# oksuman/sorting-fhe

Hardware: AMD Instinct MI355X
Metric: encrypted rank-sort homomorphic comparisons/s (N^2 per DirectSort<N>::sort) (higher is better)
Workload: dtype u64 (RNS residues, 40/60-bit primes); 1 GPU; directsort_n256_2e16; N=256, ring_dim=65536, mult_depth=34, scale_bits=40, parallelism=replicas x1

## Files before the change

include/sfhe.h:

```cpp
#ifndef SFHE_H
#define SFHE_H

#include <stddef.h>
#include <stdint.h>

#ifdef __cplusplus
extern "C" {
#endif

#define SFHE_ABI_VERSION 3

#define SFHE_OK 0
#define SFHE_EINVAL (-1)
#define SFHE_ESCHEME (-2)
#define SFHE_EDEVICE (-3)
#define SFHE_ENOTIMPL (-4)

typedef struct sfhe_ctx sfhe_ctx;
typedef struct sfhe_ct sfhe_ct;
typedef struct sfhe_sorter sfhe_sorter;

#define SFHE_FLEXIBLEAUTO 2
#define SFHE_FLEXIBLEAUTOEXT 3

// ... 4 lines not shown
    uint32_t mult_depth;
    uint32_t scaling_mod_size;
    uint32_t first_mod_size;
    uint32_t batch_size;
    uint32_t ring_dim;
    int32_t security_level;
    uint32_t num_large_digits;
    int32_t device;
    uint64_t seed;
    int32_t scaling_technique;
} sfhe_params;

int sfhe_abi_version(void);
const char* sfhe_last_error(void);
const char* sfhe_backend(void);
void sfhe_params_default(sfhe_params* p);

int sfhe_context_create(const sfhe_params* p, sfhe_ctx** out);
void sfhe_context_destroy(sfhe_ctx* c);
int sfhe_keygen(sfhe_ctx* c);
int sfhe_rotate_keygen(sfhe_ctx* c, const int32_t* idx, size_t count);
int sfhe_context_info(sfhe_ctx* c, uint32_t* ring_dim, uint32_t* mult_depth, uint32_t* num_q,
                      uint32_t* num_p, uint32_t* dnum);
int sfhe_context_primes(sfhe_ctx* c, uint64_t* out, size_t cap, size_t* count);
int sfhe_set_plaintext_cache(sfhe_ctx* c, int on);
int sfhe_set_quiet(sfhe_ctx* c, int quiet);
int sfhe_sync(sfhe_ctx* c);
int sfhe_op_stats(sfhe_ctx* c, uint64_t* counts, double* bytes, int reset);
int sfhe_bootstrap_graphs(sfhe_ctx* c, uint64_t* count);
int sfhe_encode_counts(sfhe_ctx* c, uint64_t* device, uint64_t* host);
int sfhe_decode_counts(sfhe_ctx* c, uint64_t* device, uint64_t* host);
int sfhe_tie_counts(sfhe_ctx* c, uint64_t* fused, uint64_t* composed);
int sfhe_const_term_counts(sfhe_ctx* c, uint64_t* merged, uint64_t* single, uint64_t* composed);
int sfhe_sample_counts(sfhe_ctx* c, uint64_t* device, uint64_t* host);
int sfhe_pool_bytes(sfhe_ctx* c, uint64_t* bytes);
int sfhe_live_contexts(void);
#define SFHE_KFAM_NTT 0
#define SFHE_KFAM_CONV 1
#define SFHE_KFAM_KSINNER 2
#define SFHE_KFAM_NTTKS 3
#define SFHE_KFAM_OTHER 4
#define SFHE_KFAM_ALL 5
int sfhe_kernel_timing(sfhe_ctx* c, uint32_t family, uint32_t period);
int sfhe_kernel_timing_read(sfhe_ctx* c, uint32_t family, uint64_t* launches, uint64_t* timed,
                            double* ms, double* bytes);
int sfhe_serialize_lanes(sfhe_ctx* c, int on);
int sfhe_stack_stats(sfhe_ctx* c, uint64_t* merged, uint64_t* single);
int sfhe_comm_stats_reset(sfhe_ctx* c, int timed);
int sfhe_comm_stats(sfhe_ctx* c, uint64_t* calls, double* bytes, double* ms);

int sfhe_encrypt(sfhe_ctx* c, const double* values, size_t len, uint32_t slots, uint32_t level,
                 sfhe_ct** out);
int sfhe_encrypt_batch(sfhe_ctx* c, const double* values, size_t stride, const size_t* lens, size_t count,
                       uint32_t slots, const uint32_t* levels, sfhe_ct** outs);
int sfhe_decrypt(sfhe_ctx* c, const sfhe_ct* ct, double* out, size_t cap, size_t* len);
int sfhe_decrypt_batch(sfhe_ctx* c, const sfhe_ct* const* cts, size_t count, double* out, size_t stride,
                       size_t* lens);
void sfhe_ct_free(sfhe_ct* ct);
int sfhe_ct_clone(const sfhe_ct* ct, sfhe_ct** out);
int sfhe_ct_info(const sfhe_ct* ct, uint32_t* level, uint32_t* slots, uint32_t* limbs);
int sfhe_ct_set_slots(sfhe_ct* ct, uint32_t slots);
int sfhe_ct_download(sfhe_ctx* c, const sfhe_ct* ct, uint64_t* out, size_t cap_words);

int sfhe_eval_add(sfhe_ctx* c, const sfhe_ct* a, const sfhe_ct* b, sfhe_ct** out);
int sfhe_eval_sub(sfhe_ctx* c, const sfhe_ct* a, const sfhe_ct* b, sfhe_ct** out);
int sfhe_eval_add_const(sfhe_ctx* c, const sfhe_ct* a, double k, sfhe_ct** out);
int sfhe_eval_mult_const(sfhe_ctx* c, const sfhe_ct* a, double k, sfhe_ct** out);
int sfhe_eval_mult_plain(sfhe_ctx* c, const sfhe_ct* a, const double* values, size_t len,
                         uint32_t slots, sfhe_ct** out);
int sfhe_eval_mult(sfhe_ctx* c, const sfhe_ct* a, const sfhe_ct* b, sfhe_ct** out);
int sfhe_eval_rotate(sfhe_ctx* c, const sfhe_ct* a, int32_t r, sfhe_ct** out);
int sfhe_eval_rotate_sum(sfhe_ctx* c, const sfhe_ct* const* a, const int32_t* r, size_t count, sfhe_ct** out);
int sfhe_bootstrap_setup(sfhe_ctx* c, uint32_t budget_c2s, uint32_t budget_s2c, uint32_t slots);
int sfhe_bootstrap_depth(sfhe_ctx* c, uint32_t budget_c2s, uint32_t budget_s2c, uint32_t slots, uint32_t* depth);
int sfhe_bootstrap(sfhe_ctx* c, const sfhe_ct* a, uint32_t iterations, uint32_t precision, sfhe_ct** out);
int sfhe_eval_chebyshev(sfhe_ctx* c, const sfhe_ct* x, const double* coeffs, size_t count,
                        double a, double b, sfhe_ct** out);

int sfhe_sign(sfhe_ctx* c, const sfhe_ct* x, int n, int dg, int df, sfhe_ct** out);
int sfhe_compare(sfhe_ctx* c, const sfhe_ct* a, const sfhe_ct* b, int n, int dg, int df,
                 sfhe_ct** out);
int sfhe_direct_sort_params(uint32_t N, uint32_t* mult_depth, int32_t* rotations, size_t cap,
                            size_t* count);
int sfhe_doubled_sinc_coeffs(uint32_t N, double* out, size_t cap, size_t* count);
int sfhe_sorter_create(sfhe_ctx* c, uint32_t N, int debug, sfhe_sorter** out);
int sfhe_sorter_create_rot(sfhe_ctx* c, uint32_t N, int debug, const int32_t* rotations, size_t nrot,
                           sfhe_sorter** out);
void sfhe_sorter_destroy(sfhe_sorter* s);
int sfhe_sorter_sort(sfhe_sorter* s, sfhe_ct* in, int n, int dg, int df, sfhe_ct** out);
int sfhe_sorter_rank(sfhe_sorter* s, const sfhe_ct* in, int n, int dg, int df, sfhe_ct** out);
int sfhe_sorter_place(sfhe_sorter* s, const sfhe_ct* rank, sfhe_ct* in, sfhe_ct** out);
int sfhe_sorter_sort_stable(sfhe_sorter* s, sfhe_ct* in, int n, int dg, int df, sfhe_ct** out);
int sfhe_sorter_rank_stable(sfhe_sorter* s, const sfhe_ct* in, int n, int dg, int df, sfhe_ct** out);
int sfhe_sorter_graph_nodes(const sfhe_sorter* s, uint64_t* nodes);
int sfhe_sorter_graph_ntt_time(sfhe_sorter* s, int reps, double* ms, uint64_t* launches, double* bytes);
int sfhe_sorter_graph_family_time(sfhe_sorter* s, uint32_t family, int reps, double* ms, uint64_t* launches,
                                  double* bytes);
int sfhe_sorter_sort_hybrid1(sfhe_sorter* s, sfhe_ct* in, int n, int dg, int df, sfhe_ct** out);
int sfhe_hybrid1_params(uint32_t N, uint32_t* mult_depth, int32_t* rotations, size_t cap, size_t* count);

int sfhe_sorter_sort_hybrid(sfhe_sorter* s, sfhe_ct* in, int variant, int n, int dg, int df, sfhe_ct** out);
int sfhe_hybrid_params(uint32_t N, int variant, uint32_t* mult_depth, int32_t* rotations, size_t cap,
                       size_t* count);
int sfhe_sorter_place_2n(sfhe_sorter* s, const sfhe_ct* rank, sfhe_ct* in, sfhe_ct** out);
int sfhe_sorter_sort_bitonic(sfhe_sorter* s, sfhe_ct* in, int n, int dg, int df, sfhe_ct** out);
// ... 39 lines not shown
```

sorting-fhe_amd/csrc/algo/sign.cpp:

```cpp
#include "sign.h"

#include <algorithm>
#include <cmath>
#include <cstdlib>
#include <map>
#include <vector>

using namespace lbcrypto;

namespace {

using Ct = Ciphertext<DCRTPoly>;

Ct constTermAt(const CryptoContext<DCRTPoly>& cc, const Ct& x, double c, uint32_t at) {
    const uint64_t *r0, *r1;
    std::vector<DeviceBufferPtr> keep;
    cc->RowsAt(x, at - 1, &r0, &r1, keep);
    const std::vector<const uint64_t*> i0{r0}, i1{r1};
    const std::vector<double> w{c}, sc{x->scale};
    return cc->LinearWSumRescale(i0, i1, w, at - 1, x->GetSlots(), &sc);
}

struct OddPoly {
    const CryptoContext<DCRTPoly>& cc;
// ... 18 lines not shown
        if (cnt == 1) return x->GetLevel() + 1;
        const size_t half = cnt / 2;
        return std::max(natural(half), pw[powIndex(half)]->GetLevel()) + 1;
    }
    Ct eval(const double* c, size_t cnt, uint32_t want) {
        if (cnt == 1) return constAt(c[0], std::max(x->GetLevel() + 1, want));
        const size_t half = cnt / 2, j = powIndex(half);
        const uint32_t Lp = std::max(std::max(natural(half), pw[j]->GetLevel()) + 1, want);
        Ct hi = eval(c + half, half, Lp - 1);
        Ct prod = cc->EvalMult(hi, power(j, Lp - 1));
        Ct lo = eval(c, half, Lp);
        return cc->EvalAdd(lo, prod);
    }
};

bool signBatch() {
    static const bool on = [] {
        const char* v = std::getenv("SFHE_SIGN_BATCH");
        return !v || *v != '0';
    }();
    return on;
}

struct OddPolyWaves {
    const CryptoContext<DCRTPoly>& cc;
    const Ct& x;
    const uint32_t L;
    struct Node {
        const double* c;
        size_t cnt, j;
        uint32_t Lp;
        int hi, lo;
        Ct prod, out;
    };
    std::vector<Node> nodes;
    std::vector<Ct> pw;
    std::map<std::pair<size_t, uint32_t>, Ct> aligned;

    uint32_t pwLevel(size_t j) const { return L + 1 + (uint32_t)j; }
    uint32_t natural(size_t cnt) const {
        if (cnt == 1) return L + 1;
        const size_t half = cnt / 2;
        return std::max(natural(half), pwLevel(OddPoly::powIndex(half))) + 1;
    }
    int build(const double* c, size_t cnt, uint32_t want) {
        Node nd{c, cnt, 0, 0, -1, -1, nullptr, nullptr};
        if (cnt == 1) {
            nd.Lp = std::max(L + 1, want);
        } else {
            const size_t half = cnt / 2;
            nd.j = OddPoly::powIndex(half);
            nd.Lp = std::max(std::max(natural(half), pwLevel(nd.j)) + 1, want);
            nd.hi = build(c + half, half, nd.Lp - 1);
            nd.lo = build(c, half, nd.Lp);
        }
        nodes.push_back(nd);
        return (int)nodes.size() - 1;
    }
    Ct run(const std::vector<double>& c) {
        const int root = build(c.data(), c.size(), 0);
        size_t npw = 1;
        for (size_t p = 4; p < 2 * c.size(); p *= 2) ++npw;
        cc->Settle(x);
        while (!nodes[root].out) {
            std::vector<Ct> prods;
            const size_t ready = pw.size();
            if (pw.size() < npw) {
                pw.push_back(cc->EvalSquare(pw.empty() ? x : pw.back()));
                prods.push_back(pw.back());
            }
            std::vector<std::pair<size_t, uint32_t>> align;
            for (Node& nd : nodes) {
                if (nd.cnt == 1 || nd.prod || nd.j >= ready) continue;
                const Ct* power = &pw[nd.j];
                if (pwLevel(nd.j) < nd.Lp - 1) {
                    const auto key = std::make_pair(nd.j, nd.Lp - 1);
                    auto it = aligned.find(key);
                    if (it == aligned.end()) {
                        if (std::find(align.begin(), align.end(), key) == align.end()) align.push_back(key);
                        continue;
                    }
                    power = &it->second;
                }
                if (!nodes[nd.hi].out) continue;
                nd.prod = cc->EvalMult(nodes[nd.hi].out, *power);
                prods.push_back(nd.prod);
            }
            const bool first = ready == 0;
            if (prods.empty() && align.empty() && !first)
                throw OpenFHEException("internal: odd-polynomial wave evaluation stalled");
            cc->MaterializeMany(prods, std::vector<char>(prods.size(), 0));
            if (first) {
                std::vector<std::pair<double, uint32_t>> terms;
                for (const Node& nd : nodes)
                    if (nd.cnt == 1) terms.emplace_back(nd.c[0], nd.Lp);
                const auto cts = cc->ConstTermsRescale(x, terms);
                size_t t = 0;
                for (Node& nd : nodes)
                    if (nd.cnt == 1) nd.out = cts[t++];
            }
            for (const auto& key : align) aligned[key] = cc->AdjustLevel(pw[key.first], key.second);
            for (Node& nd : nodes)
                if (nd.cnt > 1 && !nd.out && nd.prod && nodes[nd.lo].out) nd.out = cc->EvalAdd(nodes[nd.lo].out, nd.prod);
        }
        return nodes[root].out;
    }
};

Ct oddPolyFull(const CryptoContext<DCRTPoly>& cc, const Ct& x, const std::vector<double>& c) {
    if (signBatch() && c.size() > 1) {
        OddPolyWaves w{cc, x, x->GetLevel(), {}, {}, {}};
        return w.run(c);
    }
    std::vector<Ct> pw;
    pw.push_back(cc->EvalSquare(x));
    for (size_t p = 4; p < 2 * c.size(); p *= 2) pw.push_back(cc->EvalSquare(pw.back()));
    OddPoly op{cc, x, pw, {}};
    return op.eval(c.data(), c.size(), 0);
}

template <int n>
struct CompositePolys;

template <>
struct CompositePolys<3> {
    static constexpr int g_depth = 3, f_depth = 3;
    static Ct g(const Ct& x, const CryptoContext<DCRTPoly>& cc) {
        static const std::vector<double> c = {4589.0 / 1024, -16577.0 / 1024, 25614.0 / 1024,
                                              -12860.0 / 1024};
        return oddPolyFull(cc, x, c);
    }
    static Ct f(const Ct& x, const CryptoContext<DCRTPoly>& cc) {
        static const std::vector<double> c = {35.0 / 16, -35.0 / 16, 21.0 / 16, -5.0 / 16};
        return oddPolyFull(cc, x, c);
    }
};
// ... 58 lines not shown
```

sorting-fhe_amd/csrc/capi.cpp:

```cpp
#include <cstring>
#include <fstream>
#include <iostream>
#include <memory>
#include <mutex>
#include <sstream>
#include <streambuf>
#include <string>

#include "../../include/sfhe.h"
#include "algo/coefficients.h"
#include "algo/comparison.h"
#include "algo/encryption.h"
#include "algo/rotation.h"
#include "algo/sign.h"
#include "algo/sort_algo.h"
#include "algo/kway_adapter.h"
#include "core/openfhe.h"
#include "core/state.h"

using namespace lbcrypto;
using Ct = Ciphertext<DCRTPoly>;

struct sfhe_ctx {
    CryptoContext<DCRTPoly> cc;
// ... 322 lines not shown
        for (size_t k = 0; k < count; ++k) {
            const auto& v = pts[k]->GetRealPackedValue();
            if (lens) lens[k] = v.size();
            for (size_t i = 0; i < v.size() && i < stride; ++i) out[k * stride + i] = v[i];
        }
    });
}

int sfhe_decode_counts(sfhe_ctx* c, uint64_t* device, uint64_t* host) {
    REQUIRE(c && device && host, "null argument");
    auto s = c->cc->GetOpStats();
    *device = s.dev_decodes;
    *host = s.host_decodes;
    return SFHE_OK;
}

int sfhe_tie_counts(sfhe_ctx* c, uint64_t* fused, uint64_t* composed) {
    REQUIRE(c && fused && composed, "null argument");
    auto s = c->cc->GetOpStats();
    *fused = s.tie_fused;
    *composed = s.tie_composed;
    return SFHE_OK;
}

int sfhe_const_term_counts(sfhe_ctx* c, uint64_t* merged, uint64_t* single, uint64_t* composed) {
    REQUIRE(c && merged && single && composed, "null argument");
    auto s = c->cc->GetOpStats();
    *merged = s.const_merged;
    *single = s.const_single;
    *composed = s.const_composed;
    return SFHE_OK;
}

void sfhe_ct_free(sfhe_ct* ct) { delete ct; }

int sfhe_ct_clone(const sfhe_ct* ct, sfhe_ct** out) {
    REQUIRE(ct && out, "null argument");
    return guard([&] { *out = wrap(ct->ct->Clone()); });
}

int sfhe_ct_info(const sfhe_ct* ct, uint32_t* level, uint32_t* slots, uint32_t* limbs) {
    REQUIRE(ct, "null ciphertext");
    if (level) *level = ct->ct->GetLevel();
    if (slots) *slots = ct->ct->GetSlots();
    if (limbs) *limbs = ct->ct->GetNumLimbs();
    return SFHE_OK;
}

int sfhe_ct_set_slots(sfhe_ct* ct, uint32_t slots) {
    REQUIRE(ct && slots && !(slots & (slots - 1)), "slots must be a power of two");
    ct->ct->SetSlots(slots);
    return SFHE_OK;
}

int sfhe_ct_download(sfhe_ctx* c, const sfhe_ct* ct, uint64_t* out, size_t cap) {
    REQUIRE(c && ct && out, "null argument");
    const size_t n = c->cc->GetRingDimension();
    const size_t L = ct->ct->GetNumLimbs();
    REQUIRE(cap >= 2 * L * n, "output buffer too small");
    return guard([&] { c->cc->DownloadRows(ct->ct, out); });
}

#define BINOP(name, expr)                                                           \
    int name(sfhe_ctx* c, const sfhe_ct* a, const sfhe_ct* b, sfhe_ct** out) {       \
        REQUIRE(c && a && b && out, "null argument");                               \
        return guard([&] { *out = wrap(expr); });                                   \
    }
BINOP(sfhe_eval_add, c->cc->EvalAdd(a->ct, b->ct))
BINOP(sfhe_eval_sub, c->cc->EvalSub(a->ct, b->ct))
BINOP(sfhe_eval_mult, c->cc->EvalMult(a->ct, b->ct))

int sfhe_eval_add_const(sfhe_ctx* c, const sfhe_ct* a, double k, sfhe_ct** out) {
    REQUIRE(c && a && out, "null argument");
    return guard([&] { *out = wrap(c->cc->EvalAdd(a->ct, k)); });
}
int sfhe_eval_mult_const(sfhe_ctx* c, const sfhe_ct* a, double k, sfhe_ct** out) {
    REQUIRE(c && a && out, "null argument");
    return guard([&] { *out = wrap(c->cc->EvalMult(a->ct, k)); });
}
int sfhe_eval_mult_plain(sfhe_ctx* c, const sfhe_ct* a, const double* v, size_t len,
                         uint32_t slots, sfhe_ct** out) {
    REQUIRE(c && a && out && (v || !len), "null argument");
    return guard([&] {
        auto pt = c->cc->MakeCKKSPackedPlaintext(std::vector<double>(v, v + len), 1,
                                                 a->ct->GetLevel(), nullptr, slots);
        *out = wrap(c->cc->EvalMult(a->ct, pt));
    });
}
int sfhe_eval_rotate(sfhe_ctx* c, const sfhe_ct* a, int32_t r, sfhe_ct** out) {
    REQUIRE(c && a && out, "null argument");
    return guard([&] { *out = wrap(c->cc->EvalRotate(a->ct, r)); });
}
int sfhe_eval_rotate_sum(sfhe_ctx* c, const sfhe_ct* const* a, const int32_t* r, size_t count, sfhe_ct** out) {
    REQUIRE(c && a && r && out && count, "null argument");
    for (size_t k = 0; k < count; ++k) REQUIRE(a[k], "null argument");
    return guard([&] {
        std::vector<Ciphertext<DCRTPoly>> v;
        for (size_t k = 0; k < count; ++k) v.push_back(a[k]->ct);
        *out = wrap(c->cc->EvalRotateSum(v, std::vector<int32_t>(r, r + count)));
    });
}
int sfhe_bootstrap_setup(sfhe_ctx* c, uint32_t budget_c2s, uint32_t budget_s2c, uint32_t slots) {
    REQUIRE(c, "null argument");
    REQUIRE(c->keys.secretKey, "sfhe_keygen must be called first");
    return guard([&] {
        c->cc->EvalBootstrapSetup({budget_c2s, budget_s2c}, {0, 0}, slots);
        c->cc->EvalBootstrapKeyGen(c->keys.secretKey, slots);
    });
}
int sfhe_bootstrap_depth(sfhe_ctx* c, uint32_t budget_c2s, uint32_t budget_s2c, uint32_t slots, uint32_t* depth) {
    REQUIRE(c && depth, "null argument");
    return guard([&] { *depth = c->cc->GetBootstrapDepth({budget_c2s, budget_s2c}, slots); });
}
int sfhe_bootstrap(sfhe_ctx* c, const sfhe_ct* a, uint32_t iterations, uint32_t precision, sfhe_ct** out) {
    REQUIRE(c && a && out, "null argument");
    return guard([&] { *out = wrap(c->cc->EvalBootstrap(a->ct, iterations, precision)); });
}
int sfhe_eval_chebyshev(sfhe_ctx* c, const sfhe_ct* x, const double* coeffs, size_t count,
                        double a, double b, sfhe_ct** out) {
    REQUIRE(c && x && coeffs && count && out, "null argument");
    return guard([&] {
        *out = wrap(c->cc->EvalChebyshevSeriesPS(x->ct, std::vector<double>(coeffs, coeffs + count), a, b));
    });
}

int sfhe_sign(sfhe_ctx* c, const sfhe_ct* x, int n, int dg, int df, sfhe_ct** out) {
    REQUIRE(c && x && out, "null argument");
    REQUIRE(n == 3 || n == 4, "composite sign degree n must be 3 or 4");
    return guard([&] { *out = wrap(sign(x->ct, c->cc, SignFunc::CompositeSign, cfgOf(n, dg, df))); });
}

int sfhe_compare(sfhe_ctx* c, const sfhe_ct* a, const sfhe_ct* b, int n, int dg, int df,
// ... 546 lines not shown
```

sorting-fhe_amd/csrc/core/chebyshev.cpp:

```cpp
#include <algorithm>
#include <cmath>
#include <cstdio>
#include <cstdlib>
#include <map>

#include "state.h"

namespace lbcrypto {

uint32_t ChebyshevPSDepth(uint32_t d) {
    if (d <= 1) return 1;
    if (d == 2) return 2;
    static const uint32_t ub[] = {5, 13, 27, 59, 119, 247, 495, 1007, 2031, 4031, 8127, 16255, 32511, 65023};
    for (uint32_t i = 0; i < sizeof(ub) / sizeof(ub[0]); ++i)
        if (d <= ub[i]) return 3 + i;
    SFHE_THROW("Chebyshev degree too large");
}

std::vector<double> EvalChebyshevCoefficients(std::function<double(double)> func, double a,
                                              double b, uint32_t degree) {
    if (!degree) SFHE_THROW("degree must be positive");
    const double bMinusA = 0.5 * (b - a), bPlusA = 0.5 * (b + a);
    const double piByDeg = M_PI / (double)degree;
    std::vector<double> fx(degree);
// ... 15 lines not shown
    });
    return c;
}

namespace {

using Ct = Ciphertext<DCRTPoly>;
using Addend = CryptoContextImpl<DCRTPoly>::MultAddend;

struct Val {
    bool isConst = true;
    double c = 0.0;
    Ct ct;
    int node = -1;
};

bool psWaves() {
    static const bool on = [] {
        const char* v = std::getenv("SFHE_PS_WAVES");
        return !v || *v != '0';
    }();
    return on;
}

class PSEvaluator {
  public:
    PSEvaluator(CryptoContextImpl<DCRTPoly>* cc, const Ct& y, uint32_t l, uint32_t D)
        : cc(cc), l(l), k(1u << l), D(D) {
        T.resize(k + 1);
        T[1] = y;
        for (uint32_t half = 1; half < k; half *= 2) {
            const uint32_t lo = half + 1, hi = std::min(k, 2 * half);
            std::vector<Ct> as, bs;
            for (uint32_t j = lo; j <= hi; ++j) {
                as.push_back(doubled(j / 2));
                bs.push_back(j % 2 == 0 ? T[j / 2] : T[j / 2 + 1]);
            }
            uint32_t top = 0;
            for (size_t i = 0; i < as.size(); ++i) top = std::max(top, std::max(as[i]->GetLevel(), bs[i]->GetLevel()) + 1);
            if (psFma() && top <= cc->GetMultiplicativeDepth()) {
                std::vector<Addend> adds;
                for (uint32_t j = lo; j <= hi; ++j) {
                    const uint32_t lv = std::max(as[j - lo]->GetLevel(), bs[j - lo]->GetLevel()) + 1;
                    adds.push_back(j % 2 == 0 ? Addend{nullptr, 1, -1.0} : Addend{atLevel(1, lv), -1, 0.0});
                }
                if (psWaves()) {
                    auto ts = cc->EvalMultManyAdd(as, bs, adds);
                    for (uint32_t j = lo; j <= hi; ++j) T[j] = ts[j - lo];
                } else {
                    for (uint32_t j = lo; j <= hi; ++j) T[j] = cc->EvalMultAdd(as[j - lo], bs[j - lo], adds[j - lo]);
                }
                continue;
            }
            std::vector<Ct> prods;
            if (psWaves()) {
                prods = cc->EvalMultMany(as, bs);
            } else {
                for (size_t i = 0; i < as.size(); ++i) prods.push_back(cc->EvalMult(as[i], bs[i]));
            }
            for (uint32_t j = lo; j <= hi; ++j) {
                const Ct& prod = prods[j - lo];
                T[j] = (j % 2 == 0) ? cc->EvalAdd(prod, -1.0) : cc->EvalSub(prod, atLevel(1, prod->GetLevel()));
            }
        }
        giant[l] = T[k];
    }

    void precomputeLeaves(const std::vector<double>& p, uint32_t depth) {
        std::vector<std::pair<std::vector<double>, uint32_t>> leaves;
        plan(p, depth, 0, leaves);
        std::map<uint32_t, std::vector<size_t>> byLevel;
        for (size_t i = 0; i < leaves.size(); ++i) byLevel[leaves[i].second].push_back(i);
        pre.assign(leaves.size(), nullptr);
        preConst.assign(leaves.size(), 0);
        for (auto& kv : byLevel) {
            const uint32_t L = kv.first;
            std::vector<uint32_t> js;
            for (uint32_t j = 1; j <= k; ++j)
                for (size_t i : kv.second)
                    if (j < leaves[i].first.size() && leaves[i].first[j] != 0.0) {
                        js.push_back(j);
                        break;
                    }
            std::vector<const uint64_t*> ins0, ins1;
            std::vector<double> sc;
            std::vector<DeviceBufferPtr> keep;
            for (uint32_t j : js) {
                const Ct& t = T[j];
                const uint64_t *r0, *r1;
                cc->RowsAt(t, L, &r0, &r1, keep);
                ins0.push_back(r0);
// ... 224 lines not shown

    int leafSumLevel(const std::vector<double>& p, uint32_t want) const {
        if (naturalOnly()) want = 0;
        int lev = -1;
        for (uint32_t j = 1; j < p.size(); ++j)
            if (p[j] != 0.0) lev = std::max(lev, (int)T[j]->GetLevel());
        if (lev < 0) return -1;
        return std::max(lev, (int)want - 1);
    }

    static bool naturalOnly() {
        static const bool on = [] {
            const char* v = std::getenv("SFHE_PS_NATURAL");
            return v && *v == '1';
        }();
        return on;
    }

    static void trim(std::vector<double>& p) {
        while (!p.empty() && p.back() == 0.0) p.pop_back();
    }

    uint32_t powerLevel(uint32_t M) const {
        if (M <= k) return T[M]->GetLevel();
        return powerLevel(M / 2) + 1;
    }

    const Ct& power(uint32_t M) {
        if (M <= k) return T[M];
        uint32_t i = (uint32_t)__builtin_ctz(M);
        auto it = giant.find(i);
        if (it != giant.end()) return it->second;
        const Ct& half = power(M / 2);
        const Ct twice = cc->EvalAdd(half, half);
        return giant[i] = cc->EvalMultAdd(twice, half, Addend{nullptr, 1, -1.0});
    }

    const Ct& doubled(uint32_t j) {
        auto it = twice.find(j);
        if (it != twice.end()) return it->second;
        return twice[j] = cc->EvalAdd(T[j], T[j]);
    }

    const Ct& alignedPower(uint32_t M, uint32_t level) {
        const Ct& t = power(M);
        if (t->GetLevel() >= level) return t;
        auto key = std::make_pair(M, level);
        auto it = alignedPow.find(key);
        if (it != alignedPow.end()) return it->second;
        return alignedPow[key] = cc->AdjustLevel(t, level);
    }

    const Ct& atLevel(uint32_t j, uint32_t level) {
        auto key = std::make_pair(j, level);
        auto it = aligned.find(key);
        if (it != aligned.end()) return it->second;
        return aligned[key] = (T[j]->GetLevel() == level ? T[j] : cc->AdjustLevel(T[j], level));
    }

    Val leaf(const std::vector<double>& p, uint32_t want) {
        if (!pre.empty()) {
            bool any = false;
            for (uint32_t j = 1; j < p.size(); ++j) any = any || p[j] != 0.0;
            if (!any) return Val{true, p[0], nullptr};
            if (nextLeaf >= pre.size()) SFHE_THROW("internal: Chebyshev leaf plan mismatch");
            Val out;
            out.isConst = false;
            out.ct = pre[nextLeaf];
            const bool constIn = preConst[nextLeaf];
            pre[nextLeaf++] = nullptr;
            if (p[0] != 0.0 && !constIn) out.ct = cc->EvalAdd(out.ct, p[0]);
            return out;
        }
        const int lv = leafSumLevel(p, want);
// ... 2 lines not shown
        std::vector<double> w, sc;
        std::vector<DeviceBufferPtr> keep;
        for (uint32_t j = 1; j < p.size(); ++j) {
            if (p[j] == 0.0) continue;
            const Ct& t = T[j];
            const uint64_t *r0, *r1;
            cc->RowsAt(t, (uint32_t)lv, &r0, &r1, keep);
            ins0.push_back(r0);
            ins1.push_back(r1);
            w.push_back(p[j]);
            sc.push_back(t->scale);
        }
        Val out;
        out.isConst = false;
        out.ct = cc->LinearWSumRescale(ins0, ins1, w, (uint32_t)lv, T[1]->GetSlots(), &sc, p[0]);
        return out;
    }

    CryptoContextImpl<DCRTPoly>* cc;
    uint32_t l, k, D;
    std::vector<Ct> pre;
    std::vector<char> preConst;
    size_t nextLeaf = 0;
    std::vector<Ct> T;
    std::map<uint32_t, Ct> giant;
    std::map<std::pair<uint32_t, uint32_t>, Ct> aligned, alignedPow;
    std::map<uint32_t, Ct> twice;
};

void psDebugCounts(const CryptoContextImpl<DCRTPoly>* cc, const char* where) {
    if (!std::getenv("SFHE_PS_DEBUG")) return;
    uint64_t sums = 0, consts = 0, pairs = 0;
    cc->FusedSumCounts(&sums, &consts, &pairs);
    std::fprintf(stderr, "PSFMA %s | fused sums %llu | fused constants %llu | paired weighted sums %llu\n", where,
                 (unsigned long long)sums, (unsigned long long)consts, (unsigned long long)pairs);
}

}

Ciphertext<DCRTPoly> CryptoContextImpl<DCRTPoly>::EvalChebyshevSeriesPS(
    const Ciphertext<DCRTPoly>& x, const std::vector<double>& coeffs, double a, double b) {
    OpLock g(st.get());
    static const bool lazyPs = [] {
        const char* v = std::getenv("SFHE_LAZY_PS");
        return v && *v == '1';
    }();
    struct Hold {
        SfheContextState* s;
        bool on;
        ~Hold() {
            if (on) --s->lazyHold;
        }
    } hold{st.get(), !lazyPs};
    if (hold.on) ++st->lazyHold;
    std::vector<double> p(coeffs);
    while (!p.empty() && p.back() == 0.0) p.pop_back();
    if (p.empty()) SFHE_THROW("empty Chebyshev series");
    p[0] *= 0.5;
    Ciphertext<DCRTPoly> y = x;
    if (a != -1.0 || b != 1.0) {
        y = EvalMult(x, 2.0 / (b - a));
        y = EvalAdd(y, -(a + b) / (b - a));
    }
    const uint32_t d = (uint32_t)p.size() - 1;
    if (d == 0) return EvalAdd(EvalMult(y, 0.0), p[0]);
    const uint32_t D = ChebyshevPSDepth(d);
    uint32_t bestL = 1;
    double bestCost = 1e300;
// ... 112 lines not shown
```

sorting-fhe_amd/csrc/core/context.cpp:

```cpp
#include <typeindex>
#include <tuple>
#include <algorithm>
#include <atomic>
#include <cmath>
#include <cstdio>
#include <cstdlib>
#include <cstring>
#include <random>

#include "state.h"

namespace lbcrypto {

namespace {

u64 mulmod(u64 a, u64 b, u64 m) { return (u64)((u128)a * b % m); }
u64 powmod(u64 a, u64 e, u64 m) {
    u64 r = 1 % m;
    a %= m;
    while (e) {
        if (e & 1) r = mulmod(r, a, m);
        a = mulmod(a, a, m);
        e >>= 1;
    }
// ... 851 lines not shown
        const uint32_t ell = s->ellOf(level);
        if (ell < 2) SFHE_THROW("no levels left to rescale (multiplicative depth exhausted)");
        if (s->shardAt(ell)) {
            keySwitchShard(cc, d2, ell, s->relinKey, d0, d1, 1, 1);
            return rescale(cc, d0, d1, level, slots);
        }
        const DeviceBufferPtr& key = s->relinFor(ell);
        const int tier = key->ksTier;
        const uint32_t n = s->n, K = s->Kof(tier);
        const uint32_t beta = (ell + s->alpha - 1) / s->alpha;
        const size_t stride = (size_t)(ell + K) * n;
        auto acc = s->alloc(2 * stride);
        const int rowDone = modupInner(cc, acc->ptr, d2, ell, key, d0, d1, s->pModQof(tier)[ell - 1], 0, ell - 1);
        Ct out = newCt(cc, level + 1, slots);
        auto scratch = s->alloc((size_t)2 * (ell - 1) * n);
        if (f && *f && sfp_moddown_rescale_add &&
            sfp_moddown_rescale_add(s->dev, out->c0, out->c1, d0, d1, acc->ptr, stride, ell, K, s->Lq,
                                    s->moddownConvOf(tier), s->pInvModQof(tier), s->pModQof(tier),
                                    s->qInvTable[ell].data(), scratch->ptr, rowDone, f->r0, f->r1, f->sign,
                                    f->cst) == 0)
            f->done = true;
        else
            sfp_moddown_rescale(s->dev, out->c0, out->c1, d0, d1, acc->ptr, stride, ell, K, s->Lq,
                                s->moddownConvOf(tier), s->pInvModQof(tier), s->pModQof(tier),
                                s->qInvTable[ell].data(), scratch->ptr, rowDone);
        s->stats.keyswitch++;
        s->stats.rescale++;
        s->countBytes((3.0 * ell + 2.0 * beta * (ell + K)) * n * 8);
        s->countBytes(4.0 * ell * n * 8);
        return out;
    }

    static Ct multRelinRescale(CC* cc, const uint64_t* a0, const uint64_t* a1, const uint64_t* b0,
                               const uint64_t* b1, uint32_t level, uint32_t slots, Fma* f = nullptr) {
        SfheContextState* s = cc->st.get();
        const uint32_t ell = s->ellOf(level);
        if (ell < 2) SFHE_THROW("no levels left to rescale (multiplicative depth exhausted)");
        const size_t pw = s->polyWords(level);
        if (!s->shardAt(ell)) {
            const DeviceBufferPtr& key = s->relinFor(ell);
            const int tier = key->ksTier;
            const uint32_t n = s->n, K = s->Kof(tier), beta = (ell + s->alpha - 1) / s->alpha;
            const size_t stride = (size_t)(ell + K) * n;
            Ct out = newCt(cc, level + 1, slots);
            auto acc = s->alloc(2 * stride);
            auto ext = s->alloc(stride * beta);
            auto scratch = s->alloc((size_t)2 * ell * n);
            auto& convs = modupConv(cc, ell, tier);
            int rc = -1;
            if (f && *f && sfp_mult_relin_rescale_add) {
                rc = sfp_mult_relin_rescale_add(s->dev, out->c0, out->c1, a0, a1, b0, b1, ell, K, s->Lq, s->alpha,
                                                convs.data(), key->ptr, s->moddownConvOf(tier),
                                                s->pInvModQof(tier), s->pModQof(tier), s->qInvTable[ell].data(),
                                                acc->ptr, ext->ptr, scratch->ptr, f->r0, f->r1, f->sign, f->cst);
                if (rc == 0) f->done = true;
            }
            if (rc != 0)
                rc = sfp_mult_relin_rescale(s->dev, out->c0, out->c1, a0, a1, b0, b1, ell, K, s->Lq, s->alpha,
                                            convs.data(), key->ptr, s->moddownConvOf(tier), s->pInvModQof(tier),
                                            s->pModQof(tier), s->qInvTable[ell].data(), acc->ptr, ext->ptr,
                                            scratch->ptr);
            if (rc == 0) {
                s->stats.keyswitch++;
                s->stats.rescale++;
                s->countBytes((3.0 * ell + 2.0 * beta * (ell + K)) * n * 8);
                s->countBytes(4.0 * ell * n * 8);
                return out;
            }
        }
        auto t = s->alloc(3 * pw);
        uint64_t* d0 = t->ptr;
        uint64_t* d1 = d0 + pw;
        uint64_t* d2 = d1 + pw;
        sfp_tensor(s->dev, d0, d1, d2, a0, a1, b0, b1, s->qmap(ell));
        return relinRescale(cc, d0, d1, d2, level, slots, f);
    }

    static std::vector<Ct> multRelinRescaleMany(CC* cc, const std::vector<const CiphertextImpl<DCRTPoly>*>& a,
                                                const std::vector<const CiphertextImpl<DCRTPoly>*>& b, uint32_t level,
                                                const std::vector<uint32_t>& slots, std::vector<Fma>* fs = nullptr) {
        SfheContextState* s = cc->st.get();
        const size_t cnt = a.size();
        const uint32_t ell = s->ellOf(level);
        std::vector<Ct> out(cnt);
        if (ell < 2) SFHE_THROW("no levels left to rescale (multiplicative depth exhausted)");
        const DeviceBufferPtr& key = s->relinFor(ell);
        const int tier = key->ksTier;
        const uint32_t n = s->n, K = s->Kof(tier), beta = (ell + s->alpha - 1) / s->alpha;
        const size_t stride = (size_t)(ell + K) * n;
        auto& convs = modupConv(cc, ell, tier);
        size_t done = 0;
        {
        BatchScope bs(cc, s->shardAt(ell) ? 0 : (uint32_t)cnt);
        if (bs) {
            for (; done < cnt; ++done) {
                out[done] = newCt(cc, level + 1, slots[done]);
                auto acc = s->alloc(2 * stride);
                auto ext = s->alloc(stride * beta);
                auto scratch = s->alloc((size_t)2 * ell * n);
                bs.lane((uint32_t)done);
                Fma* f = fs && (*fs)[done] ? &(*fs)[done] : nullptr;
                int rc = -1;
                if (f && sfp_mult_relin_rescale_add) {
                    rc = sfp_mult_relin_rescale_add(s->dev, out[done]->c0, out[done]->c1, a[done]->c0, a[done]->c1,
                                                    b[done]->c0, b[done]->c1, ell, K, s->Lq, s->alpha, convs.data(),
                                                    key->ptr, s->moddownConvOf(tier), s->pInvModQof(tier),
                                                    s->pModQof(tier), s->qInvTable[ell].data(), acc->ptr, ext->ptr,
                                                    scratch->ptr, f->r0, f->r1, f->sign, f->cst);
                    if (rc == 0) f->done = true;
                }
                if (rc != 0)
                    rc = sfp_mult_relin_rescale(s->dev, out[done]->c0, out[done]->c1, a[done]->c0, a[done]->c1,
                                                b[done]->c0, b[done]->c1, ell, K, s->Lq, s->alpha, convs.data(),
                                                key->ptr, s->moddownConvOf(tier), s->pInvModQof(tier),
                                                s->pModQof(tier), s->qInvTable[ell].data(), acc->ptr, ext->ptr,
                                                scratch->ptr);
                if (rc != 0) break;
                s->stats.keyswitch++;
                s->stats.rescale++;
                s->countBytes((3.0 * ell + 2.0 * beta * (ell + K)) * n * 8);
                s->countBytes(4.0 * ell * n * 8);
            }
        }
        }
        for (size_t i = done; i < cnt; ++i)
            out[i] = multRelinRescale(cc, a[i]->c0, a[i]->c1, b[i]->c0, b[i]->c1, level, slots[i],
                                      fs ? &(*fs)[i] : nullptr);
        return out;
    }

    static void innerAndModDown(CC* cc, const uint64_t* ext, size_t stride, uint32_t beta,
                                uint32_t ell, const DeviceBufferPtr& key, uint64_t* out0,
                                uint64_t* out1, int add0, int add1, uint32_t gal = 0) {
        SfheContextState* s = cc->st.get();
        if (s->shardAt(ell)) {
            if (gal) SFHE_THROW("internal: a permuted inner product at a sharded level");
            return innerModDownShard(s, ext, stride, beta, ell, key, out0, out1, add0, add1);
        }
        const int tier = key->ksTier;
        const uint32_t n = s->n, K = s->Kof(tier);
        const size_t accStride = (size_t)(ell + K) * n;
        if (stride != accStride) SFHE_THROW("internal: extended digits of another special-prime tier");
        auto acc = s->alloc(2 * accStride);
        if (gal)
            sfp_ks_inner_aut(s->dev, acc->ptr, acc->ptr + accStride, ext, stride, key->ptr, beta, ell, K, s->Lq, gal);
        else
            sfp_ks_inner(s->dev, acc->ptr, acc->ptr + accStride, ext, stride, key->ptr, beta, ell, K, s->Lq);
        auto scratch = s->alloc((size_t)2 * ell * n);
        sfp_moddown2(s->dev, out0, out1, acc->ptr, accStride, ell, K, s->Lq, s->moddownConvOf(tier),
                     s->pInvModQof(tier), add0, add1, scratch->ptr, 0);
    }

    static std::vector<sfp_conv*>& modupConv(CC* cc, uint32_t ell, int tier = -1) {
        SfheContextState* s = cc->st.get();
        auto& cache = tier < 0 ? s->modupConv : s->tiers[(size_t)tier].modupConv;
        auto it = cache.find(ell);
        if (it != cache.end()) return it->second;
        std::vector<sfp_conv*> v;
        const uint32_t K = s->Kof(tier);
        uint32_t beta = (ell + s->alpha - 1) / s->alpha;
// ... 643 lines not shown
        for (size_t g : grp) {
            used[g] = true;
            defs.push_back(SfheInternal::takeDeferred(*a[idx[g]], true));
            auto* m = static_cast<DeferredMacPlain*>(defs.back().get());
            for (auto& b : m->pins) s->dep(b.get());
            pts.insert(pts.end(), m->pts.begin(), m->pts.end());
        }
        SfheInternal::encodeBatch(cc, pts, level);
        std::vector<const uint64_t*> mm;
        for (auto& p : pts) mm.push_back(SfheInternal::encoded(cc, p, level));
        const uint32_t ell = s->ellOf(level);
        const size_t pw = s->polyWords(level);
        std::vector<DeviceBufferPtr> bufs;
        std::vector<uint64_t*> o0, o1;
        for (uint32_t g = 0; g < ng; ++g) {
            bufs.push_back(s->alloc(2 * pw));
            o0.push_back(bufs.back()->ptr);
            o1.push_back(bufs.back()->ptr + pw);
        }
        const auto* x = static_cast<DeferredMacPlain*>(defs[0].get());
        if (sfp_mac_plain2_multi(s->dev, o0.data(), o1.data(), x->x0.data(), x->x1.data(), mm.data(), nin, ng,
                                 s->qmap(ell)) != 0)
            for (uint32_t g = 0; g < ng; ++g)
                sfp_mac_plain2(s->dev, o0[g], o1[g], x->x0.data(), x->x1.data(), mm.data() + (size_t)g * nin, nin,
                               s->qmap(ell));
        for (uint32_t g = 0; g < ng; ++g) SfheInternal::adoptPending(*a[idx[grp[g]]], bufs[g], o0[g], o1[g]);
    }
}

struct DeferredRelin : DeferredOp {
    DeviceBufferPtr pa, pb;
    const uint64_t *a0, *a1, *b0, *b1;
    uint32_t level, slots;
    void sync(SfheContextState* s) override {
        s->dep(pa.get());
        s->dep(pb.get());
    }
    void run(CCI* cc, CtI& ct, bool pending) override {
        SfheContextState* s = cc->state();
        s->dep(pa.get());
        s->dep(pb.get());
        if (!pending) {
            SfheInternal::adopt(ct, SfheInternal::multRelinRescale(cc, a0, a1, b0, b1, level, slots));
            return;
        }
        const size_t pw = s->polyWords(level);
        auto t = s->alloc(3 * pw);
        uint64_t* d0 = t->ptr;
        uint64_t* d1 = d0 + pw;
        uint64_t* d2 = d1 + pw;
        sfp_tensor(s->dev, d0, d1, d2, a0, a1, b0, b1, s->qmap(s->ellOf(level)));
        SfheInternal::keySwitch(cc, d2, s->ellOf(level), s->relinFor(s->ellOf(level)), d0, d1, 1, 1);
        SfheInternal::adoptPending(ct, t, d0, d1);
    }
};
}


static std::atomic<int> g_liveContexts{0};
int CryptoContextImpl<DCRTPoly>::LiveContexts() { return g_liveContexts.load(); }

void SfheCheckLayout(uint64_t callerStamp) {
    const uint64_t mine = SfheFacadeLayout();
    if (callerStamp == mine) return;
    char b[160];
    std::snprintf(b, sizeof b, "caller stamp %016llx, library stamp %016llx (facade ABI version %d)",
                  (unsigned long long)callerStamp, (unsigned long long)mine, SFHE_FACADE_ABI_VERSION);
    SFHE_THROW(std::string("the engine headers this program was compiled against do not match the library's "
                           "(object layouts differ; rebuild the program against the installed headers): ") + b);
}

CryptoContextImpl<DCRTPoly>::CryptoContextImpl(const CCParams<CryptoContextCKKSRNS>& p)
    : st(new SfheContextState) {
    SfheContextState& s = *st;
// ... 298 lines not shown
    s->opMu.unlock();
    return false;
}

uint32_t CryptoContextImpl<DCRTPoly>::BatchWidth() const { return batchWidth(); }

void CryptoContextImpl<DCRTPoly>::BatchLane(uint32_t i) {
    OpLock g(st.get());
    if (st->batchDepth) sfp_batch_lane(st->dev, i);
}

void CryptoContextImpl<DCRTPoly>::EndBatch() {
    OpLock g(st.get());
    SfheContextState* s = st.get();
    if (!s->batchDepth) return;
    sfp_batch_end(s->dev);
    std::lock_guard<std::mutex> pg(s->poolMu);
    --s->batchDepth;
    for (auto& e : s->batchFree) s->poolReturn(e.words, e.ptr, e.lane, e.region, s->myLane());
    s->batchFree.clear();
    s->opMu.unlock();
}

void CryptoContextImpl<DCRTPoly>::MaterializeMany(const std::vector<Ciphertext<DCRTPoly>>& cts,
                                                  const std::vector<char>& pendingOk) {
    if (cts.size() != pendingOk.size()) SFHE_THROW("MaterializeMany: flag count mismatch");
    OpLock g(st.get());
    SfheContextState* s = st.get();
    struct Item {
        uint32_t level;
        std::type_index kind;
        bool pending;
        size_t ct;
        bool like(const Item& o) const { return level == o.level && kind == o.kind && pending == o.pending; }
    };
    std::vector<Item> items;
    for (size_t i = 0; i < cts.size(); ++i) {
        const auto& c = cts[i];
        if (!c || (!c->def && !(c->pend && !pendingOk[i]))) continue;
        const DeferredOp* d = c->def.get();
        items.push_back({c->level ? c->level - 1 : 0, d ? std::type_index(typeid(*d)) : std::type_index(typeid(void)),
                         pendingOk[i] != 0, i});
    }
    std::stable_sort(items.begin(), items.end(), [](const Item& a, const Item& b) {
        return std::tie(a.level, a.kind, a.pending) < std::tie(b.level, b.kind, b.pending);
    });
    const size_t w = batchWidth();
    for (size_t b0 = 0, b1; b0 < items.size(); b0 = b1) {
        const bool lone = items[b0].kind == std::type_index(typeid(void));
        for (b1 = b0 + 1; !lone && b1 < items.size() && b1 - b0 < w && items[b1].like(items[b0]);) ++b1;
        const bool shard = s->shardAt(s->ellOf(items[b0].level));
        for (size_t k = b0; k < b1; ++k) {
            auto& c = *cts[items[k].ct];
            if (c.def)
                c.def->sync(s);
            else
                s->dep(c.buf.get());
        }
        BatchScope bs(this, shard ? 0u : (uint32_t)(b1 - b0));
        for (size_t k = b0; k < b1; ++k) {
            bs.lane((uint32_t)(k - b0));
            SfheInternal::materialize(*cts[items[k].ct], items[k].pending);
        }
    }
}

void CryptoContextImpl<DCRTPoly>::SetPlaintextCache(bool on) {
    OpLock g(st.get());
    st->ptCacheOn = on;
    if (!on) {
        st->ptCache.clear();
        st->ptCacheBytes = 0;
    }
}

CryptoContextImpl<DCRTPoly>::OpStats CryptoContextImpl<DCRTPoly>::GetOpStats() const {
    OpStats o = st->stats;
    std::lock_guard<std::mutex> g(st->poolMu);
// ... 759 lines not shown
    if (ell < 3) SFHE_THROW("no levels left (the tie term consumes two levels)");
    const uint32_t slots = std::max(a->slots, W->slots);
    const uint64_t* w = SfheInternal::encodedNextScale(this, W, level);
    const auto kr = SfheInternal::constResidues(s, k * a->scale * s->scale[level + 1], ell);
    const size_t pw = s->polyWords(level);
    const sfp_limbs m = s->qmap(ell);
    auto t = s->alloc(3 * pw);
    uint64_t* d0 = t->ptr;
    uint64_t* d1 = d0 + pw;
    uint64_t* d2 = d1 + pw;
    const char* knob = std::getenv("SFHE_TIE_FUSED");
    const bool fused = sfp_tie_tensor && !(knob && *knob == '0') && !s->shardAt(ell) &&
                       sfp_tie_tensor(s->dev, d0, d1, d2, a->c0, a->c1, w, kr.data(), m) == 0;
    if (fused) {
        s->stats.tie_fused++;
    } else {
        auto u = s->alloc(2 * pw);
        uint64_t* u0 = u->ptr;
        uint64_t* u1 = u0 + pw;
        sfp_mul(s->dev, u0, a->c0, w, m);
        sfp_mul(s->dev, u1, a->c1, w, m);
        sfp_add_const(s->dev, u0, u0, kr.data(), m);
        sfp_tensor(s->dev, d0, d1, d2, a->c0, a->c1, u0, u1, m);
        s->stats.tie_composed++;
    }
    s->stats.ptmult++;
    s->stats.tensor++;
    s->countBytes(12.0 * ell * s->n * 8);
    auto r = SfheInternal::relinRescale(this, d0, d1, d2, level, slots);
    return SfheInternal::traced(this, SfheInternal::rescale(this, r->c0, r->c1, level + 1, slots), "EvalTieTerm");
}

std::vector<Ciphertext<DCRTPoly>> CryptoContextImpl<DCRTPoly>::EvalMultMany(
    const std::vector<Ciphertext<DCRTPoly>>& a0, const std::vector<Ciphertext<DCRTPoly>>& b0) {
    OpLock g(st.get());
    SfheContextState* s = st.get();
    if (a0.size() != b0.size()) SFHE_THROW("operand count mismatch");
    const size_t cnt = a0.size();
    std::vector<Ciphertext<DCRTPoly>> out(cnt);
    if (cnt < 2 || !SfheInternal::fusedRescale()) {
        for (size_t i = 0; i < cnt; ++i) out[i] = EvalMult(a0[i], b0[i]);
        return out;
    }
    if (!s->relinKey) SFHE_THROW("EvalMultKeyGen must be called before EvalMult");
    std::vector<Ciphertext<DCRTPoly>> A(a0), B(b0);
    for (size_t i = 0; i < cnt; ++i) {
        SfheInternal::deps(s, {&a0[i], &b0[i]});
        SfheInternal::align(this, A[i], B[i]);
        if (s->ellOf(A[i]->level) < 2) SFHE_THROW("no levels left (multiplicative depth exhausted)");
        s->stats.tensor++;
        s->countBytes(7.0 * s->ellOf(A[i]->level) * s->n * 8);
    }
    for (size_t i = 0; i < cnt;) {
        size_t j = i + 1;
        while (j < cnt && j - i < batchWidth() && A[j]->level == A[i]->level) ++j;
        std::vector<const CiphertextImpl<DCRTPoly>*> pa, pb;
        std::vector<uint32_t> slots;
        for (size_t k = i; k < j; ++k) {
            pa.push_back(A[k].get());
            pb.push_back(B[k].get());
            slots.push_back(std::max(A[k]->slots, B[k]->slots));
        }
        auto r = SfheInternal::multRelinRescaleMany(this, pa, pb, A[i]->level, slots);
        for (size_t k = i; k < j; ++k) out[k] = SfheInternal::traced(this, r[k - i], "EvalMult");
        i = j;
    }
    return out;
}

namespace {
Ciphertext<DCRTPoly> addAfter(CryptoContextImpl<DCRTPoly>* cc, Ciphertext<DCRTPoly> prod,
                              const CryptoContextImpl<DCRTPoly>::MultAddend& add) {
    if (add.r) prod = add.sign < 0 ? cc->EvalSub(prod, add.r) : cc->EvalAdd(prod, add.r);
    if (add.c != 0.0) prod = cc->EvalAdd(prod, add.c);
    return prod;
}
}

bool CryptoContextImpl<DCRTPoly>::multAddFusable(const Ciphertext<DCRTPoly>& a, const Ciphertext<DCRTPoly>& b,
                                                 const MultAddend& add) const {
    SfheContextState* s = st.get();
    if (!psFma() || !SfheInternal::fusedRescale() || SfheInternal::lazy(s) || !s->relinKey) return false;
    if (!add.r && add.c == 0.0) return false;
    if (SfheInternal::isLazy(a) || SfheInternal::isLazy(b)) return false;
    const uint32_t level = std::max(a->level, b->level);
    const uint32_t ell = s->ellOf(level);
    if (ell < 2 || s->shardAt(ell) || level + 1 > s->L) return false;
    if (add.r) {
        const auto& r = add.r;
        if (SfheInternal::isLazy(r) || r->level != level + 1 || r->scale != s->scale[level + 1] ||
            r->c1 - r->c0 != (ptrdiff_t)s->polyWords(level + 1))
            return false;
    }
    return true;
}

Ciphertext<DCRTPoly> CryptoContextImpl<DCRTPoly>::EvalMultAdd(const Ciphertext<DCRTPoly>& a0,
                                                             const Ciphertext<DCRTPoly>& b0,
                                                             const MultAddend& add) {
    OpLock g(st.get());
    if (!multAddFusable(a0, b0, add)) return addAfter(this, EvalMult(a0, b0), add);
    SfheContextState* s = st.get();
    SfheInternal::deps(s, {&a0, &b0, &add.r});
    auto a = a0, b = b0;
    SfheInternal::align(this, a, b);
    const uint32_t ell = s->ellOf(a->level), slots = std::max(a->slots, b->slots);
    s->stats.tensor++;
    s->countBytes(7.0 * ell * s->n * 8);
    std::vector<uint64_t> k;
    SfheInternal::Fma f;
    if (add.r) {
        f.r0 = add.r->c0;
        f.r1 = add.r->c1;
        f.sign = add.sign;
    }
    if (add.c != 0.0) {
        k = SfheInternal::constResidues(s, add.c * s->scale[a->level + 1], ell - 1);
        f.cst = k.data();
    }
    auto out = SfheInternal::traced(
        this, SfheInternal::multRelinRescale(this, a->c0, a->c1, b->c0, b->c1, a->level, slots, &f), "EvalMult");
    if (!f.done) return addAfter(this, out, add);
    SfheInternal::countFused(s, add, ell - 1);
    return out;
}

std::vector<Ciphertext<DCRTPoly>> CryptoContextImpl<DCRTPoly>::EvalMultManyAdd(
    const std::vector<Ciphertext<DCRTPoly>>& a0, const std::vector<Ciphertext<DCRTPoly>>& b0,
    const std::vector<MultAddend>& adds) {
    OpLock g(st.get());
    SfheContextState* s = st.get();
    if (a0.size() != b0.size() || a0.size() != adds.size()) SFHE_THROW("operand count mismatch");
    const size_t cnt = a0.size();
    std::vector<Ciphertext<DCRTPoly>> out(cnt);
    if (cnt < 2) {
        for (size_t i = 0; i < cnt; ++i) out[i] = EvalMultAdd(a0[i], b0[i], adds[i]);
        return out;
    }
    if (!psFma() || !SfheInternal::fusedRescale() || SfheInternal::lazy(s)) {
        out = EvalMultMany(a0, b0);
        for (size_t i = 0; i < cnt; ++i) out[i] = addAfter(this, out[i], adds[i]);
        return out;
    }
    if (!s->relinKey) SFHE_THROW("EvalMultKeyGen must be called before EvalMult");
    std::vector<Ciphertext<DCRTPoly>> A(a0), B(b0);
    std::vector<char> fuse(cnt);
    for (size_t i = 0; i < cnt; ++i) {
        fuse[i] = multAddFusable(a0[i], b0[i], adds[i]);
        SfheInternal::deps(s, {&a0[i], &b0[i]});
        if (fuse[i]) SfheInternal::deps(s, {&adds[i].r});
        SfheInternal::align(this, A[i], B[i]);
        if (s->ellOf(A[i]->level) < 2) SFHE_THROW("no levels left (multiplicative depth exhausted)");
        s->stats.tensor++;
        s->countBytes(7.0 * s->ellOf(A[i]->level) * s->n * 8);
    }
    for (size_t i = 0; i < cnt;) {
        size_t j = i + 1;
        while (j < cnt && j - i < batchWidth() && A[j]->level == A[i]->level) ++j;
        const uint32_t level = A[i]->level, ell = s->ellOf(level);
        std::vector<const CiphertextImpl<DCRTPoly>*> pa, pb;
        std::vector<uint32_t> slots;
        std::vector<SfheInternal::Fma> fs(j - i);
        std::vector<std::vector<uint64_t>> ks(j - i);
        for (size_t k = i; k < j; ++k) {
            pa.push_back(A[k].get());
            pb.push_back(B[k].get());
            slots.push_back(std::max(A[k]->slots, B[k]->slots));
            if (!fuse[k]) continue;
            SfheInternal::Fma& f = fs[k - i];
            if (adds[k].r) {
                f.r0 = adds[k].r->c0;
                f.r1 = adds[k].r->c1;
                f.sign = adds[k].sign;
            }
            if (adds[k].c != 0.0) {
                ks[k - i] = SfheInternal::constResidues(s, adds[k].c * s->scale[level + 1], ell - 1);
                f.cst = ks[k - i].data();
            }
        }
        auto r = SfheInternal::multRelinRescaleMany(this, pa, pb, level, slots, &fs);
        for (size_t k = i; k < j; ++k) {
            out[k] = SfheInternal::traced(this, r[k - i], "EvalMult");
            if (fs[k - i].done)
                SfheInternal::countFused(s, adds[k], ell - 1);
            else
                out[k] = addAfter(this, out[k], adds[k]);
        }
        i = j;
    }
    return out;
}

Ciphertext<DCRTPoly> CryptoContextImpl<DCRTPoly>::EvalMultAddPlain(
    const std::vector<Ciphertext<DCRTPoly>>& a, const std::vector<Plaintext>& p) {
    OpLock g(st.get());
    SfheInternal::depsv(st.get(), a);
    SfheContextState* s = st.get();
    if (a.empty() || a.size() != p.size()) SFHE_THROW("operand count mismatch");
    uint32_t level = 0, slots = 0;
    for (size_t i = 0; i < a.size(); ++i) {
        level = std::max(level, a[i]->level);
        slots = std::max(slots, std::max(a[i]->slots, p[i]->slots));
    }
    const uint32_t ell = s->ellOf(level);
    if (ell < 2) SFHE_THROW("no levels left (multiplicative depth exhausted)");
    std::vector<Ciphertext<DCRTPoly>> al(a.size());
    std::vector<const uint64_t*> x0, x1, m;
    for (size_t i = 0; i < a.size(); ++i) {
        al[i] = SfheInternal::adjust(this, a[i], level);
        x0.push_back(al[i]->c0);
        x1.push_back(al[i]->c1);
    }
    s->stats.ptmult += a.size();
    if (SfheInternal::lazy(s)) {
        auto op = std::make_shared<DeferredMacPlain>();
        for (auto& c : al) op->pins.push_back(c->buf);
        op->x0 = x0;
        op->x1 = x1;
        op->pts = p;
        op->level = level;
        op->slots = slots;
        s->countBytes((3.0 * a.size() + 2.0) * ell * s->n * 8);
        return SfheInternal::deferredCt(this, level + 1, slots, op);
// ... 948 lines not shown
```

sorting-fhe_amd/csrc/core/openfhe.h:

```cpp
#pragma once

#include <algorithm>
#include <charconv>
#include <complex>
#include <cstddef>
#include <locale>
#include <fstream>
#include <cstdint>
#include <functional>
#include <iostream>
#include <map>
#include <memory>
#include <mutex>
#include <set>
#include <stdexcept>
#include <string>
#include <thread>
#include <vector>

#include "prims.h"

namespace lbcrypto {

using usint = uint32_t;
// ... 256 lines not shown
    Ciphertext<DCRTPoly> EvalAdd(const Plaintext& p, const Ciphertext<DCRTPoly>& a) {
        return EvalAdd(a, p);
    }
    void EvalAddInPlace(Ciphertext<DCRTPoly>& a, const Ciphertext<DCRTPoly>& b);
    void EvalAddInPlace(Ciphertext<DCRTPoly>& a, double c);
    void EvalAddInPlace(Ciphertext<DCRTPoly>& a, const Plaintext& p);
    Ciphertext<DCRTPoly> EvalSub(const Ciphertext<DCRTPoly>& a, const Ciphertext<DCRTPoly>& b);
    Ciphertext<DCRTPoly> EvalSub(const Ciphertext<DCRTPoly>& a, double c) { return EvalAdd(a, -c); }
    Ciphertext<DCRTPoly> EvalSub(double c, const Ciphertext<DCRTPoly>& a);
    Ciphertext<DCRTPoly> EvalSub(const Ciphertext<DCRTPoly>& a, const Plaintext& p);
    Ciphertext<DCRTPoly> EvalSub(const Plaintext& p, const Ciphertext<DCRTPoly>& a);
    void EvalSubInPlace(Ciphertext<DCRTPoly>& a, const Ciphertext<DCRTPoly>& b);
    void EvalSubInPlace(Ciphertext<DCRTPoly>& a, double c) { EvalAddInPlace(a, -c); }
    Ciphertext<DCRTPoly> EvalNegate(const Ciphertext<DCRTPoly>& a);
    void EvalNegateInPlace(Ciphertext<DCRTPoly>& a);
    Ciphertext<DCRTPoly> EvalAddMany(const std::vector<Ciphertext<DCRTPoly>>& v);

    Ciphertext<DCRTPoly> EvalMult(const Ciphertext<DCRTPoly>& a, const Ciphertext<DCRTPoly>& b);
    Ciphertext<DCRTPoly> EvalMult(const Ciphertext<DCRTPoly>& a, double c);
    Ciphertext<DCRTPoly> EvalMult(double c, const Ciphertext<DCRTPoly>& a) { return EvalMult(a, c); }
    Ciphertext<DCRTPoly> EvalMult(const Ciphertext<DCRTPoly>& a, const Plaintext& p);
    Ciphertext<DCRTPoly> EvalMult(const Plaintext& p, const Ciphertext<DCRTPoly>& a) {
        return EvalMult(a, p);
    }
    void EvalMultInPlace(Ciphertext<DCRTPoly>& a, double c);
    void EvalMultInPlace(Ciphertext<DCRTPoly>& a, const Plaintext& p);
    Ciphertext<DCRTPoly> EvalMultAndRelinearize(const Ciphertext<DCRTPoly>& a,
                                                const Ciphertext<DCRTPoly>& b) {
        return EvalMult(a, b);
    }
    Ciphertext<DCRTPoly> EvalSquare(const Ciphertext<DCRTPoly>& a);
    Ciphertext<DCRTPoly> EvalTieTerm(const Ciphertext<DCRTPoly>& s, const Plaintext& W, double k);
    std::vector<Ciphertext<DCRTPoly>> EvalMultMany(const std::vector<Ciphertext<DCRTPoly>>& a,
                                                   const std::vector<Ciphertext<DCRTPoly>>& b);
    struct MultAddend {
        Ciphertext<DCRTPoly> r;
        int sign = 1;
        double c = 0.0;
    };
    Ciphertext<DCRTPoly> EvalMultAdd(const Ciphertext<DCRTPoly>& a, const Ciphertext<DCRTPoly>& b,
                                     const MultAddend& add);
    std::vector<Ciphertext<DCRTPoly>> EvalMultManyAdd(const std::vector<Ciphertext<DCRTPoly>>& a,
                                                      const std::vector<Ciphertext<DCRTPoly>>& b,
                                                      const std::vector<MultAddend>& adds);
    Ciphertext<DCRTPoly> EvalMultAddPlain(const std::vector<Ciphertext<DCRTPoly>>& a,
                                          const std::vector<Plaintext>& p);

    Ciphertext<DCRTPoly> EvalRotate(const Ciphertext<DCRTPoly>& a, int32_t r);
    Ciphertext<DCRTPoly> EvalAtIndex(const Ciphertext<DCRTPoly>& a, int32_t r) {
        return EvalRotate(a, r);
    }
    std::shared_ptr<FastRotationPrecomp> EvalFastRotationPrecompute(const Ciphertext<DCRTPoly>& a);
    Ciphertext<DCRTPoly> EvalFastRotation(const Ciphertext<DCRTPoly>& a, int32_t r, uint32_t m,
                                          const std::shared_ptr<FastRotationPrecomp>& pre);
    Ciphertext<DCRTPoly> EvalRotateSum(const std::vector<Ciphertext<DCRTPoly>>& a,
                                       const std::vector<int32_t>& r);
    Ciphertext<DCRTPoly> EvalRotMultAddHoisted(
        const std::vector<Ciphertext<DCRTPoly>>& a,
        const std::vector<std::vector<std::pair<int32_t, Plaintext>>>& terms);

    Ciphertext<DCRTPoly> EvalChebyshevSeriesPS(const Ciphertext<DCRTPoly>& x,
                                               const std::vector<double>& coeffs, double a,
                                               double b);
    Ciphertext<DCRTPoly> EvalChebyshevSeries(const Ciphertext<DCRTPoly>& x,
                                             const std::vector<double>& coeffs, double a,
                                             double b) {
        return EvalChebyshevSeriesPS(x, coeffs, a, b);
    }
    Ciphertext<DCRTPoly> EvalChebyshevFunction(std::function<double(double)> f,
                                               const Ciphertext<DCRTPoly>& x, double a, double b,
                                               uint32_t degree);
    Ciphertext<DCRTPoly> EvalPolyLinear(const Ciphertext<DCRTPoly>& x,
// ... 272 lines not shown
```

sorting-fhe_amd/csrc/core/state.h:

```cpp
#pragma once
#include <algorithm>
#include <atomic>
#include <cmath>
#include <cstdlib>
#include <cstring>
#include <map>
#include <mutex>
#include <thread>
#include <unordered_map>
#include <unordered_set>
#include <vector>

#include "modarith.h"
#include "openfhe.h"

namespace lbcrypto {

class DeviceBuffer {
  public:
    DeviceBuffer(SfheContextState* s, uint64_t* p, size_t w, int l, uint64_t r)
        : st(s), ptr(p), words(w), lane(l), region(r) {}
    ~DeviceBuffer();
    SfheContextState* st;
    uint64_t* ptr;
// ... 95 lines not shown
        int lane;
        uint64_t region;
    };
    uint32_t batchDepth = 0;
    std::thread::id batchThread;
    std::vector<BatchFreed> batchFree;
    void poolReturn(size_t words, uint64_t* p, int lane, uint64_t region, int freer);
    std::map<size_t, std::vector<uint64_t*>> forkPool;
    int lane = 0;
    int forkedLanes = 0;
    uint64_t region = 0;
    uint64_t regionCount = 0;
    uint64_t laneSeq[SFP_MAX_LANES] = {};
    uint64_t synced[SFP_MAX_LANES][SFP_MAX_LANES] = {};
    uint64_t regionDepWaits = 0;
    void laneWait(int waiter, int waitee);
    int myLane() const;
    void setMyLane(int l);
    void dep(DeviceBuffer* b);
    void wrote(DeviceBuffer* b);
    size_t poolBytes = 0;

    std::recursive_mutex opMu;

    bool ptCacheOn = true;
    size_t ptCacheBytes = 0;
    size_t ptCacheLimit = (size_t)48 << 30;
    std::unordered_map<uint64_t, std::vector<PtCacheEntry>> ptCache;

    bool capturing = false;
    uint64_t captureEpoch = 0, epochCount = 0;
    uint32_t lazyHold = 0;
    uint64_t fusedSums = 0, fusedConsts = 0, pairedWsums = 0;
    std::set<uint64_t> abandonedEpochs;
    std::vector<std::pair<uint64_t*, size_t>> capAllocs;
    std::unordered_map<uint64_t*, bool> graphOwned;

    std::atomic<uint64_t> seedCounter{1};
    uint64_t seed = 0;
    CryptoContextImpl<DCRTPoly>::OpStats stats;

    int rank = 0, world = 1;
    int bgroup = 0, bgroups = 1;
    bool bgatherAtOne = false;
    bool sharded = false;
    uint32_t tailLimbs = 0;
    bool fullScope = false;
    std::vector<DeviceBufferPtr> scopeKeep;
    sfp_key_geom kgeom{};
    uint32_t keyRows() const { return kgeom.rows ? kgeom.rows : Lq + K; }
    std::map<uint32_t, std::vector<sfp_conv*>> modupConvShard;
    std::map<uint32_t, std::vector<std::pair<sfp_conv*, sfp_conv*>>> modupConvSplit;
    sfp_conv* moddownConvShard = nullptr;

    uint32_t ellOf(uint32_t level) const { return Lq - level; }
    double preScale(uint32_t level) const { return scale[level] * (double)primes[ellOf(level)]; }
    uint32_t owned(uint32_t count) const {
        return (uint32_t)rank < count ? (count - rank + world - 1) / world : 0;
    }
    bool shardAt(uint32_t ell) const { return sharded && ell > tailLimbs; }
    uint32_t rows(uint32_t ell) const { return shardAt(ell) ? owned(ell) : ell; }
    uint32_t prows(uint32_t ell) const { return shardAt(ell) ? owned(K) : K; }
    uint32_t qprime(uint32_t i, uint32_t ell) const { return shardAt(ell) ? rank + i * world : i; }
    uint32_t qprimeShard(uint32_t i) const { return rank + i * world; }
    sfp_limbs shardMap(uint32_t ell) const {
        return sfp_limbs{owned(ell), owned(ell), 0, (uint32_t)rank, (uint32_t)world};
// ... 26 lines not shown
        s_->sharded = sharded_;
        s_->fullScope = was_;
        if (!was_) s_->scopeKeep.clear();
    }

  private:
    SfheContextState* s_;
    int rank_, world_;
    bool sharded_, was_;
};

inline uint32_t batchWidth() {
    static const uint32_t w = [] {
        const char* v = std::getenv("SFHE_BATCH_WIDTH");
        const long x = v && *v ? std::strtol(v, nullptr, 10) : SFP_BATCH_MAX;
        return (uint32_t)std::max(2L, std::min<long>(x, SFP_BATCH_MAX));
    }();
    return w;
}

inline bool psFma() {
    static const bool on = [] {
        const char* v = std::getenv("SFHE_PS_FMA");
        return !v || *v != '0';
    }();
    return on;
}

inline bool constTerms() {
    const char* v = std::getenv("SFHE_CONST_TERMS");
    return !v || *v != '0';
}

class OpLock {
  public:
    explicit OpLock(SfheContextState* s) : s_(s), g_(s->opMu) {
        s_->lane = s_->myLane();
        sfp_set_lane(s_->dev, s_->lane);
    }

  private:
    SfheContextState* s_;
    std::lock_guard<std::recursive_mutex> g_;
};

static inline uint64_t sf_splitmix64(uint64_t x) {
    x += 0x9E3779B97F4A7C15ULL;
    x = (x ^ (x >> 30)) * 0xBF58476D1CE4E5B9ULL;
    x = (x ^ (x >> 27)) * 0x94D049BB133111EBULL;
    return x ^ (x >> 31);
}

int ckks_encode(const std::vector<std::complex<double>>& v, uint32_t slots, uint32_t n,
                double scale, std::vector<int64_t>& coeffs);
void ckks_decode(const std::vector<double>& coeffs, uint32_t slots, uint32_t n,
                 std::vector<std::complex<double>>& out);
void ckks_encoder_tables(uint32_t n, const uint64_t** rot, const double** ksi);

}
```

sorting-fhe_amd/csrc/hip/prims_hip.hip:

```cpp
#include <hip/hip_runtime.h>
#include <dlfcn.h>
#include <rccl/rccl.h>

#include <algorithm>
#include <cstdio>
#include <cstdlib>
#include <cstring>
#include <functional>
#include <map>
#include <memory>
#include <mutex>
#include <unordered_set>
#include <unordered_map>
#include <string>
#include <type_traits>
#include <vector>

#include "../modarith.h"
#include "../prims.h"

#define SFP_CHECK(call)                                                     \
    do {                                                                    \
        hipError_t e_ = (call);                                             \
        if (e_ != hipSuccess) record(d, #call, e_);                          \
// ... 606 lines not shown
struct RowPtr {
    const u64* base;
    long long ps, is;
};
struct RowGroup {
    uint32_t P, R;
    sfp_limbs pm;
    RowPtr src, dst, copy, ein, eout;
    uint32_t copyByAlpha;
    uint32_t alpha;
    uint32_t skipEll;
    uint32_t lift, liftPrime;
    uint32_t epi, addMask;
    RowPtr eadd;
    const u64 *tA0, *tA1, *tB0, *tB1;
    RowPtr pre, emul;
    const u64 *k, *kS, *k2, *k2S, *liftSub, *preK, *preKS, *emK, *emKS;
    const u64* cy;
    const double *cmD, *cmQ, *chD, *chQ;
    const u64* cmI;
    uint32_t cRows, cBig;
    union {
        struct {
            const u64 *postK, *postKS;
            const double *postD, *postQ;
        };
        struct {
            RowPtr esum;
            const u64* ecst;
        };
    };
    const struct MdColArgs* md;
    uint32_t esumNeg;
};

template <class T, int NG>
struct ArgSet {
    T a[NG];
    uint32_t start[NG];
    uint32_t inter;
};
template <class T, int NG>
__device__ __forceinline__ uint32_t argSel(const ArgSet<T, NG>& S, uint32_t& row) {
    const uint32_t y = blockIdx.y;
    if (NG == 1) {
        row = y;
        return 0;
    }
    if (S.inter) {
        row = y / NG;
        return y % NG;
    }
    uint32_t sel = 0;
#pragma unroll
    for (int i = 1; i < NG; ++i)
        if (y >= S.start[i]) sel = (uint32_t)i;
    row = y - S.start[sel];
    return sel;
}
template <int NG>
using RowGroupSet = ArgSet<RowGroup, NG>;
static_assert(sizeof(RowGroupSet<8>) + 96 <= 4096, "eight row groups by value exceed the kernel-argument limit");

__device__ __forceinline__ u64* rowAt(const RowPtr& r, uint32_t p, uint32_t i) {
    return const_cast<u64*>(r.base) + p * r.ps + i * r.is;
}

#ifdef SFHE_NTT_TRACE
constexpr int kTraceSlots = 256;
__device__ unsigned long long g_nttTrace[kTraceSlots][4][8];
__device__ unsigned long long g_mdrsTrace[kTraceSlots][8];
#define NTT_MARK(i)                                                          \
    {                                                                        \
        const unsigned long long t_ = clock64();                             \
        tacc[(i)] += t_ - tprev;                                             \
        tprev = t_;                                                          \
    }
#else
#define NTT_MARK(i)
#endif

template <bool INV, bool COL, int LE, int TILE, int NG = 1, bool CONV = false>
__global__ __launch_bounds__(TILE >> LE) void k_ntt(const RowGroupSet<NG> GS, const sf_barrett* __restrict__ bar,
                                                  const u64* __restrict__ tw, const u64* __restrict__ twS,
                                                  const u64* __restrict__ ninv,
                                                  const u64* __restrict__ ninvS, uint32_t logn,
                                                  const double* __restrict__ twD,
                                                  const double* __restrict__ qinvD,
                                                  const double* __restrict__ ninvD,
                                                  const double* __restrict__ ninvQ, int useFp,
                                                  const double* __restrict__ rowD) {
    __shared__ u64 s[TILE];
    __shared__ u64 tW[COL ? kNttColTw : 1], tX[COL ? kNttColTw : 1];
#ifdef SFHE_NTT_TRACE
    unsigned long long tprev = clock64(), tacc[6] = {0, 0, 0, 0, 0, 0};
#endif
    constexpr bool FIRST = (COL != INV);
    const uint32_t n = 1u << logn;
    const uint32_t logR = logn - 8;
    uint32_t rid;
    const RowGroup& G = GS.a[argSel(GS, rid)];
    const uint32_t pp = rid / G.R, ii = rid % G.R;
    if (G.skipEll && ii >= G.alpha * pp && ii < min(G.alpha * (pp + 1), G.skipEll)) return;
    const uint32_t prime = primeOf(G.pm, ii);
    NttTile T;
    T.logn = logn;
    T.d = COL ? logR : 8u;
    T.logC = COL ? (uint32_t)__builtin_ctz(TILE) - logR : 0u;
    T.C = 1u << T.logC;
    const uint32_t tile = (gridDim.x & 7) ? blockIdx.x : (blockIdx.x & 7) * (gridDim.x >> 3) + (blockIdx.x >> 3);
    T.c0 = COL ? tile * T.C : 0u;
    T.r0 = COL ? 0u : tile * (TILE / 256);
    const uint32_t S0 = COL ? 0u : logR;
// ... 118 lines not shown
    const u64 q = bar[prime].q;
    const bool fp = useFp && q < kFpPrimeBound;
    const bool rowPf = kPfBuild && fp;
    if constexpr (kPfBuild)
        if (rowPf) rowTwFinish(PW, RT, (double)q, qinvD[prime]);

    const u64* gw = fp ? gwD : gwI;
    if (COL) {
#pragma unroll
        for (int c = 0; c < kColPer; ++c) {
            const uint32_t e = threadIdx.x + c * NT;
            if (e < colTw) {
                tW[e] = fp ? cwD[c] : cwI[c];
                if (!fp) tX[e] = cwX[c];
            }
        }
    }
    const u64* rw = COL ? tW : gw;
    const u64* rx = COL ? tX : gx;
    u64* cp = nullptr;
    if (FIRST && G.copy.base)
        cp = G.copyByAlpha ? const_cast<u64*>(G.copy.base) + (ii / G.alpha) * G.copy.ps + ii * G.copy.is
                           : rowAt(G.copy, pp, ii);

#pragma unroll
    for (int k = 0; k < NPAIR; ++k) {
        const uint32_t e = 2 * (threadIdx.x + k * NT);
        const size_t g = tileOff(k);
        ulonglong2 x = xr[k];
        if (FIRST) {
            if (cp) *reinterpret_cast<ulonglong2*>(cp + g) = x;
            if (pre) {
                const ulonglong2 m = mr[k];
                x.x = bmul(x.x, m.x, LB);
                x.y = bmul(x.y, m.y, LB);
            }
            if (preK) {
                x.x = sf_mul_shoup(x.x, pk, pkS, q);
                x.y = sf_mul_shoup(x.y, pk, pkS, q);
            }
            if (G.lift) {
                u64 r0 = sf_reduce128(x.x, 0, &LB), r1 = sf_reduce128(x.y, 0, &LB);
                if (x.x > lhalf) r0 = sf_sub(r0, lsub, q);
                if (x.y > lhalf) r1 = sf_sub(r1, lsub, q);
                x.x = r0;
                x.y = r1;
            }
        }
        if (fp) {
            s[ldsSw(e)] = __double_as_longlong(u2d(x.x));
            s[ldsSw(e + 1)] = __double_as_longlong(u2d(x.y));
        } else {
            s[ldsSw(e)] = x.x;
            s[ldsSw(e + 1)] = x.y;
        }
    }
    __syncthreads();
    NTT_MARK(0);
    const uint32_t nr = (T.d + LE - 1) / LE;
    if constexpr (kPfBuild) {
        if (rowPf) {
#pragma unroll
            for (int ri = 0; ri < kPfRounds; ++ri) {
                const int r = INV ? kPfRounds - 1 - ri : ri;
                nttRoundFP<INV, false, 2, 2, TILE, true, 8>(reinterpret_cast<double*>(s), T, S0, 2 * r,
                                                            (double)q, nullptr, qinvD[prime], PW + 3 * r);
// ... 67 lines not shown
            }
        } else if (!FIRST) {
            if (scale) {
                x.x = sf_mul_shoup_lazy(x.x, ni, niS, q);
                x.y = sf_mul_shoup_lazy(x.y, ni, niS, q);
            } else {
                x.x = x.x >= 2 * q ? x.x - 2 * q : x.x;
                x.y = x.y >= 2 * q ? x.y - 2 * q : x.y;
            }
            x.x = x.x >= q ? x.x - q : x.x;
            x.y = x.y >= q ? x.y - q : x.y;
        }
        if (epi) {
            ulonglong2 a = *reinterpret_cast<const ulonglong2*>(ein + g);
            if (emul) {
                const ulonglong2 m = *reinterpret_cast<const ulonglong2*>(emul + g);
                a.x = bmul(a.x, m.x, EB);
                a.y = bmul(a.y, m.y, EB);
            }
            if (emK) {
                a.x = sf_mul_shoup(a.x, emk, emkS, q);
                a.y = sf_mul_shoup(a.y, emk, emkS, q);
            }
            x.x = sf_mul_shoup(sf_sub(a.x, x.x, q), ek, ekS, q);
            x.y = sf_mul_shoup(sf_sub(a.y, x.y, q), ek, ekS, q);
            if ((G.addMask >> pp) & 1u) {
                const ulonglong2 o = *reinterpret_cast<const ulonglong2*>(out + g);
                x.x = sf_add(x.x, o.x, q);
                x.y = sf_add(x.y, o.y, q);
            }
            if (ead || tens) {
                ulonglong2 o;
                if (tens) {
                    const ulonglong2 a0 = *reinterpret_cast<const ulonglong2*>(G.tA0 + trow + g);
                    const ulonglong2 b0 = *reinterpret_cast<const ulonglong2*>(G.tB0 + trow + g);
                    if (pp == 0) {
                        o.x = bmul(a0.x, b0.x, EB);
                        o.y = bmul(a0.y, b0.y, EB);
                    } else {
                        const ulonglong2 a1 = *reinterpret_cast<const ulonglong2*>(G.tA1 + trow + g);
                        const ulonglong2 b1 = *reinterpret_cast<const ulonglong2*>(G.tB1 + trow + g);
                        Acc t{0, 0}, u{0, 0};
                        macc(t, a0.x, b1.x);
                        macc(t, a1.x, b0.x);
                        macc(u, a0.y, b1.y);
                        macc(u, a1.y, b0.y);
                        o.x = sf_reduce128_acc(t.lo, t.hi, &EB);
                        o.y = sf_reduce128_acc(u.lo, u.hi, &EB);
                    }
                } else {
                    o = *reinterpret_cast<const ulonglong2*>(ead + g);
                }
                x.x = sf_add(x.x, sf_mul_shoup(o.x, ek2, ek2S, q), q);
                x.y = sf_add(x.y, sf_mul_shoup(o.y, ek2, ek2S, q), q);
            }
            if (esm) {
                const ulonglong2 r = *reinterpret_cast<const ulonglong2*>(esm + g);
                x.x = G.esumNeg ? sf_sub(x.x, r.x, q) : sf_add(x.x, r.x, q);
                x.y = G.esumNeg ? sf_sub(x.y, r.y, q) : sf_add(x.y, r.y, q);
            }
            if (ecs) {
                x.x = sf_add(x.x, ecs, q);
                x.y = sf_add(x.y, ecs, q);
            }
        }
        *reinterpret_cast<ulonglong2*>(out + g) = x;
    }
    NTT_MARK(5);
#ifdef SFHE_NTT_TRACE
    if (threadIdx.x == 0) {
        auto& slot = g_nttTrace[(blockIdx.x + blockIdx.y * gridDim.x) % kTraceSlots][INV * 2 + COL];
        for (int i = 0; i < 6; ++i) atomicAdd(&slot[i], tacc[i]);
        atomicAdd(&slot[7], 1ull);
    }
// ... 270 lines not shown
            if (emul) a = bmul(a, emul[x], EB);
            if (emK) a = sf_mul_shoup(a, emk, emkS, q);
            v = sf_mul_shoup(sf_sub(a, v, q), ek, ekS, q);
            if ((G.addMask >> pp) & 1u) v = sf_add(v, out[x], q);
            if (ead) v = sf_add(v, sf_mul_shoup(ead[x], ek2, ek2S, q), q);
            if (esm) v = G.esumNeg ? sf_sub(v, esm[x], q) : sf_add(v, esm[x], q);
            if (ecs) v = sf_add(v, ecs, q);
        }
        out[x] = v;
    }
}


enum EwOp { EW_ADD, EW_SUB, EW_NEG, EW_MUL, EW_MULADD, EW_MULC, EW_ADDC };

struct KsArgs {
    const u64* in;
    const u64* inMul;
    const u64* ext;
    long long extStride;
    const u64* key;
    uint32_t keyRows, keyQ;
    u64* acc0;
    u64* acc1;
    const u64* fold0;
    const u64* fold1;
    u64 foldK;
    const u64 *fa0, *fa1, *fb0, *fb1;
    uint32_t ell, Lq, alpha, beta;
    int accum;
    uint32_t invFrom;
    const u64 *itw, *itwS;
    const double* itwD;
};

template <int LE, int TILE, int NG = 1>
__global__ __launch_bounds__(TILE >> LE) void k_ntt_ks(const ArgSet<KsArgs, NG> AS, const sf_barrett* __restrict__ bar,
                                                     const u64* __restrict__ tw, const u64* __restrict__ twS,
                                                     uint32_t logn, const double* __restrict__ twD,
                                                     const double* __restrict__ qinvD, int useFp,
                                                     const double* __restrict__ rowD) {
    __shared__ u64 s[2 * TILE];
    constexpr int NT = TILE >> LE;
    constexpr int NPAIR = (1 << LE) / 2;
    const uint32_t n = 1u << logn;
    const uint32_t logR = logn - 8;
    uint32_t t;
    const KsArgs& A = AS.a[argSel(AS, t)];
    const uint32_t prime = t < A.ell ? t : A.Lq + (t - A.ell);
    const sf_barrett B = loadBar(bar, prime);
    const u64 q = B.q;
    const bool fp = useFp && q < kFpPrimeBound;
    NttTile T;
    T.logn = logn;
    T.d = 8u;
    T.logC = 0;
    T.C = 1;
    const uint32_t tile = (gridDim.x & 7) ? blockIdx.x : (blockIdx.x & 7) * (gridDim.x >> 3) + (blockIdx.x >> 3);
    T.c0 = 0;
    T.r0 = tile * (TILE / 256);
    const uint32_t S0 = logR;
    const u64* gw = fp ? reinterpret_cast<const u64*>(twD) + (size_t)prime * n : tw + (size_t)prime * n;
    const u64* gx = twS + (size_t)prime * n;
    constexpr bool kPfBuild = LE == 2;
    constexpr int kPfRounds = 4;
#ifndef SFHE_KS_PW_LOOP
// ... 34 lines not shown
        using AccT = std::conditional_t<FP, double, Acc>;
        AccT a0[2 * NPAIR], a1[2 * NPAIR];
#pragma unroll
        for (int w = 0; w < 2 * NPAIR; ++w) {
            if constexpr (FP) a0[w] = a1[w] = 0.0;
            else a0[w] = a1[w] = Acc{0, 0};
        }
        auto term = [&](AccT& acc, auto x, u64 w) {
            if constexpr (FP) {
                const double wd = u2d(w);
                double y;
                if constexpr (std::is_same_v<decltype(x), u64>) y = u2d(x);
                else y = x;
                acc += fpMulMod(y, wd, wd * qi, qd);
            } else {
                macc(acc, (u64)x, w);
            }
        };
        for (uint32_t j = 0; j < A.beta; ++j) {
            const bool own = t < A.ell && t >= j * A.alpha && t < min((j + 1) * A.alpha, A.ell);
            std::conditional_t<FP, double, u64> v[2 * NPAIR];
            const u64* kb = A.key + (size_t)j * 2 * A.keyRows * n + (size_t)kr * n + rowOff;
            const u64* ka = kb + (size_t)A.keyRows * n;
            ulonglong2 kb2[NPAIR], ka2[NPAIR];
            if (own) {
                const u64* src = A.in + (size_t)t * n + rowOff;
                const u64* mul = A.inMul ? A.inMul + (size_t)t * n + rowOff : nullptr;
#pragma unroll
                for (int k = 0; k < NPAIR; ++k) {
                    const uint32_t e = 2 * (threadIdx.x + k * NT);
                    ulonglong2 x = *reinterpret_cast<const ulonglong2*>(src + e);
                    if (mul) {
                        const ulonglong2 m = *reinterpret_cast<const ulonglong2*>(mul + e);
                        x.x = bmul(x.x, m.x, B);
                        x.y = bmul(x.y, m.y, B);
                    }
                    if constexpr (FP) {
                        v[2 * k] = u2d(x.x);
                        v[2 * k + 1] = u2d(x.y);
                    } else {
                        v[2 * k] = x.x;
                        v[2 * k + 1] = x.y;
                    }
                }
#pragma unroll
                for (int k = 0; k < NPAIR; ++k) {
                    const uint32_t e = 2 * (threadIdx.x + k * NT);
                    kb2[k] = *reinterpret_cast<const ulonglong2*>(kb + e);
                    ka2[k] = *reinterpret_cast<const ulonglong2*>(ka + e);
                }
            } else {
                const u64* src = A.ext + j * A.extStride + (size_t)t * n + rowOff;
                ulonglong2 xs[NPAIR];
#pragma unroll
                for (int k = 0; k < NPAIR; ++k)
                    xs[k] = *reinterpret_cast<const ulonglong2*>(src + 2 * (threadIdx.x + k * NT));
                if constexpr (FP && SFHE_KS_PW_LOOP) loadPW(PW);
#pragma unroll
                for (int k = 0; k < NPAIR; ++k) {
                    const uint32_t e = 2 * (threadIdx.x + k * NT);
                    kb2[k] = *reinterpret_cast<const ulonglong2*>(kb + e);
                    ka2[k] = *reinterpret_cast<const ulonglong2*>(ka + e);
                }
                __syncthreads();
#pragma unroll
                for (int k = 0; k < NPAIR; ++k) {
// ... 45 lines not shown
                        x1 = x1 >= q ? x1 - q : x1;
                        v[2 * k] = x0;
                        v[2 * k + 1] = x1;
                    }
                }
            }
#pragma unroll
            for (int k = 0; k < NPAIR; ++k) {
                const ulonglong2 b2 = kb2[k];
                const ulonglong2 a2 = ka2[k];
                term(a0[2 * k], v[2 * k], b2.x);
                term(a0[2 * k + 1], v[2 * k + 1], b2.y);
                term(a1[2 * k], v[2 * k], a2.x);
                term(a1[2 * k + 1], v[2 * k + 1], a2.y);
            }
        }
        ulonglong2 prev[2][NPAIR];
        if (A.accum) {
#pragma unroll
            for (int k = 0; k < NPAIR; ++k) {
                const uint32_t e = 2 * (threadIdx.x + k * NT);
                prev[0][k] = *reinterpret_cast<const ulonglong2*>(o0 + e);
                prev[1][k] = *reinterpret_cast<const ulonglong2*>(o1 + e);
            }
        }
        const bool fold = (A.fold0 || A.fa0) && t == A.ell - 1;
        if (inv) __syncthreads();
#pragma unroll
        for (int k = 0; k < NPAIR; ++k) {
            const uint32_t e = 2 * (threadIdx.x + k * NT);
            if (fold) {
                if (A.fa0) {
                    const size_t ro = (size_t)t * n + rowOff + e;
                    const ulonglong2 x0 = *reinterpret_cast<const ulonglong2*>(A.fa0 + ro);
                    const ulonglong2 x1 = *reinterpret_cast<const ulonglong2*>(A.fa1 + ro);
                    const ulonglong2 y0 = *reinterpret_cast<const ulonglong2*>(A.fb0 + ro);
                    const ulonglong2 y1 = *reinterpret_cast<const ulonglong2*>(A.fb1 + ro);
                    if constexpr (FP) {
                        const double fk = u2d(A.foldK), fkq = fk * qi;
                        const double qx0 = u2d(x0.x), qy0 = u2d(x0.y), qx1 = u2d(x1.x), qy1 = u2d(x1.y);
                        const double b0x = u2d(y0.x), b0y = u2d(y0.y), b1x = u2d(y1.x), b1y = u2d(y1.y);
                        const double f0x = fpMulMod(qx0, b0x, b0x * qi, qd), f0y = fpMulMod(qy0, b0y, b0y * qi, qd);
                        const double f1x = fpMulMod(qx0, b1x, b1x * qi, qd) + fpMulMod(qx1, b0x, b0x * qi, qd);
                        const double f1y = fpMulMod(qy0, b1y, b1y * qi, qd) + fpMulMod(qy1, b0y, b0y * qi, qd);
                        a0[2 * k] += fpMulMod(f0x, fk, fkq, qd);
                        a0[2 * k + 1] += fpMulMod(f0y, fk, fkq, qd);
                        a1[2 * k] += fpMulMod(f1x, fk, fkq, qd);
                        a1[2 * k + 1] += fpMulMod(f1y, fk, fkq, qd);
                    } else {
                        Acc tt{0, 0}, uu{0, 0};
                        macc(tt, x0.x, y1.x);
                        macc(tt, x1.x, y0.x);
                        macc(uu, x0.y, y1.y);
                        macc(uu, x1.y, y0.y);
                        macc(a0[2 * k], bmul(x0.x, y0.x, B), A.foldK);
                        macc(a0[2 * k + 1], bmul(x0.y, y0.y, B), A.foldK);
                        macc(a1[2 * k], sf_reduce128_acc(tt.lo, tt.hi, &B), A.foldK);
                        macc(a1[2 * k + 1], sf_reduce128_acc(uu.lo, uu.hi, &B), A.foldK);
                    }
                } else {
                    const ulonglong2 f0 = *reinterpret_cast<const ulonglong2*>(A.fold0 + (size_t)t * n + rowOff + e);
                    const ulonglong2 f1 = *reinterpret_cast<const ulonglong2*>(A.fold1 + (size_t)t * n + rowOff + e);
                    term(a0[2 * k], f0.x, A.foldK);
                    term(a0[2 * k + 1], f0.y, A.foldK);
                    term(a1[2 * k], f1.x, A.foldK);
                    term(a1[2 * k + 1], f1.y, A.foldK);
                }
            }
// ... 3900 lines not shown
    A.copyByAlpha = 1;
    A.alpha = alpha;
    RowGroup B = rowsOf(beta, ell + K, sfp_limbs{ell + K, ell, Lq, 0});
    B.src = B.dst = RowPtr{ext, stride, (long long)n};
    B.skipEll = ell;
    B.alpha = alpha;
    const ModUpPlan* P = modupPlan(d, convs, ell, K, alpha);
    if (P) planInto(P, A, B, scr);
    nttRows(d, A, 1);
    if (!P) {
        ConvJobs J;
        bool fpOk = true;
        for (uint32_t j = 0; j < beta; ++j) {
            J.j[j] = convJob(convs[j], ext + j * stride, scr + (size_t)j * alpha * n, convs[j]->nt, 0);
            fpOk = fpOk && convs[j]->fpOk;
        }
        convLaunch(d, J, beta, fpOk);
    }
    nttRows(d, B, 0);
}

static bool ksFuse() {
    static const bool on = [] {
        const char* v = std::getenv("SFHE_KS_FUSE");
        return !v || *v != '0';
    }();
    return on;
}

static void modupInnerCore(sfp_dev* d, uint64_t* acc0, uint64_t* acc1, const uint64_t* in, const uint64_t* inMul,
                           uint32_t ell, uint32_t K, uint32_t Lq, uint32_t alpha, const sfp_conv* const* convs,
                           const uint64_t* key, const uint64_t* fold0, const uint64_t* fold1,
                           const uint64_t* const* T, uint64_t foldK, int accum, uint32_t invFrom, uint64_t* ext,
                           uint64_t* scr, int phases = 3) {
    const uint32_t n = d->n;
    const uint32_t beta = (ell + alpha - 1) / alpha;
    const long long stride = (long long)(ell + K) * n;
    if (phases & 1) {
    RowGroup A = rowsOf(1, ell, sfp_limbs{ell, ell, 0, 0});
    A.src = RowPtr{in, 0, (long long)n};
    A.dst = RowPtr{scr, 0, (long long)n};
    if (inMul) A.pre = RowPtr{inMul, 0, (long long)n};
    RowGroup B = rowsOf(beta, ell + K, sfp_limbs{ell + K, ell, Lq, 0});
    B.src = B.dst = RowPtr{ext, stride, (long long)n};
    B.skipEll = ell;
    B.alpha = alpha;
    const ModUpPlan* P = modupPlan(d, convs, ell, K, alpha);
    if (P) planInto(P, A, B, scr);
    nttRows(d, A, 1);
    if (!P) {
        ConvJobs J;
        bool fpOk = true;
        for (uint32_t j = 0; j < beta; ++j) {
            J.j[j] = convJob(convs[j], ext + j * stride, scr + (size_t)j * alpha * n, convs[j]->nt, 0);
            fpOk = fpOk && convs[j]->fpOk;
        }
        convLaunch(d, J, beta, fpOk);
    }
    nttRows(d, B, 0, 1);
    }
    if (!(phases & 2)) return;
    KsArgs a;
    std::memset(&a, 0, sizeof a);
    a.in = in;
    a.inMul = inMul;
    a.ext = ext;
    a.extStride = stride;
    a.key = key;
    a.keyRows = d->kg.rows ? d->kg.rows : Lq + K;
    a.keyQ = d->kg.rows ? d->kg.pstart : Lq;
    a.acc0 = acc0;
    a.acc1 = acc1;
    a.fold0 = fold0;
    a.fold1 = fold1;
    if (T) {
        a.fa0 = T[0];
        a.fa1 = T[1];
        a.fb0 = T[2];
        a.fb1 = T[3];
    }
    a.foldK = foldK;
    a.ell = ell;
    a.Lq = Lq;
    a.alpha = alpha;
    a.beta = beta;
    a.accum = accum;
    a.invFrom = invFrom;
    a.itw = d->ipsi;
    a.itwS = d->ipsiS;
    a.itwD = d->ipsiD;
    const uint32_t rows = ell + K;
    const size_t total = (size_t)rows * n;
    const bool t1k = rows <= 64 && n <= 1024u * 128u;
    timedLaunch(d, SFP_FAM_NTTKS, 8.0 * total * (3.0 * beta + (accum ? 4.0 : 2.0)), [&] {
        ArgSet<KsArgs, 1> AS;
        AS.a[0] = a;
        AS.start[0] = 0;
        AS.inter = 0;
        const int fp = nttFp();
        const dim3 g(n / (t1k ? 1024u : (uint32_t)kNttTile), rows);
        const int threads = (t1k ? 1024 : kNttTile) >> 2;
        auto k1 = t1k ? k_ntt_ks<2, 1024> : k_ntt_ks<2, kNttTile>;
        StackRec r;
        r.go = [=](hipStream_t s_) {
            hipLaunchKernelGGL(k1, g, dim3(threads), 0, s_, AS, d->bar, d->psi, d->psiS, d->logn, d->psiD, d->qinvD,
                               fp, d->rowD);
        };
        if (d->stackOn) {
            auto P = std::make_shared<KsPay>();
            P->a = a;
            P->rows = rows;
            P->g = g;
            P->threads = threads;
            P->useFp = fp;
// ... 194 lines not shown
    B.ein = RowPtr{acc, (long long)accStride, (long long)n};
    B.eout = RowPtr{out0, (long long)(out1 - out0), (long long)n};
    u64 kS[SFP_MAX_LIMBS];
    for (uint32_t i = 0; i < ell; ++i) kS[i] = sf_shoup_precomp(pinv[i], d->hbar[i].q);
    B.k = devConst(d, pinv, ell);
    B.kS = devConst(d, kS, ell);
    nttRows(d, B, 0);
}

static bool mdrsiOn() {
    static const bool on = [] {
        const char* v = std::getenv("SFHE_MDRSI");
        return !v || *v != '0';
    }();
    return on;
}

struct EpiAdd {
    const uint64_t *r0 = nullptr, *r1 = nullptr;
    int sign = 1;
    const uint64_t* cst = nullptr;
};
static void epiAddInto(sfp_dev* d, RowGroup& B, const EpiAdd& e, uint32_t npoly, uint32_t rows) {
    if (e.r0) {
        B.esum = RowPtr{e.r0, e.r1 ? (long long)(e.r1 - e.r0) : 0, (long long)d->n};
        B.esumNeg = e.sign < 0 ? 1u : 0u;
    }
    if (e.cst) B.ecst = devConst(d, e.cst, (size_t)npoly * rows);
}

static void moddownRescaleCore(sfp_dev* d, uint64_t* out0, uint64_t* out1, const uint64_t* d0, const uint64_t* d1,
                               const uint64_t* const* T, uint64_t* acc, size_t accStride, uint32_t ell, uint32_t K,
                               uint32_t Lq, const sfp_conv* c, const uint64_t* pinv, const uint64_t* pmod,
                               const uint64_t* qlinv, uint64_t* scr, int rowDone, const EpiAdd& ea = EpiAdd{}) {
    const uint32_t n = d->n, l = ell - 1;
    if (ell < 2 || ell > SFP_MAX_LIMBS || !c || c->ns > (uint32_t)kMaxConvSrc || c->nt < ell ||
        !limbsOk(d, sfp_limbs{K + 1, 1, Lq, l}, "moddown_rescale")) {
        record(d, "moddown_rescale", hipErrorInvalidValue);
        return;
    }
    RowGroup A = rowsOf(2, K + 1, sfp_limbs{K + 1, 1, Lq, l});
    A.src = A.dst = RowPtr{acc + (size_t)l * n, (long long)accStride, (long long)n};
    MdrsArgs M;
    std::memset(&M, 0, sizeof M);
    for (int p = 0; p < 2; ++p) {
        const u64* ap = acc + (size_t)p * accStride;
        M.j[p] = MdrsJob{ap + (size_t)ell * n, ap, scr + (size_t)p * l * n};
    }
    u64 lsub[SFP_MAX_LIMBS], k1[SFP_MAX_LIMBS], k1S[SFP_MAX_LIMBS], k2S[SFP_MAX_LIMBS];
    const u64 ql = d->hbar[l].q;
    for (uint32_t i = 0; i < l; ++i) {
        const u64 q = d->hbar[i].q;
        lsub[i] = ql % q;
        k1[i] = (u64)((unsigned __int128)pinv[i] * qlinv[i] % q);
        k1S[i] = sf_shoup_precomp(k1[i], q);
        k2S[i] = sf_shoup_precomp(qlinv[i], q);
    }
    const MdColArgs* md = mdColArgs(d, c, l, true, l, Lq, pmod, lsub, pinv[l], A);
    nttRows(d, A, 1, rowDone ? 2 : 3);
    if (!md) {
        M.sidx = c->src;
        M.inv = c->inv;
        M.mod = c->mod;
        M.sprod = c->sprod;
        M.pmod = devConst(d, pmod, l);
        M.lsub = devConst(d, lsub, l);
        M.pinvl = pinv[l];
// ... 48 lines not shown
                         : c->ns <= 16           ? k_mdrsi<16>
                                                 : k_mdrsi<kMaxConvSrc>;
            StackRec r;
            r.go = [=](hipStream_t s_) { hipLaunchKernelGGL(k, g, dim3(kThreads), 0, s_, M, d->bar, d->qinvD, d->logn); };
            if (d->stackOn) {
                auto P = std::make_shared<MdrsPay>();
                P->M = M;
                P->g = g;
                P->k = reinterpret_cast<ConvKern>(k);
                r.cls = STK_MDRS;
                r.key = stkKey((const void*)k, g.x, g.z);
                r.pay = std::move(P);
            }
            issueRec(d, std::move(r));
        });
        checkLaunch(d, "conv_mdrs");
    }
    RowGroup B = rowsOf(2, l, sfp_limbs{l, l, 0, 0});
    B.src = B.dst = RowPtr{scr, (long long)l * n, (long long)n};
    if (md) {
        B.md = md;
        B.copy = RowPtr{acc + (size_t)ell * n, (long long)accStride, (long long)n};
        B.pre = RowPtr{acc + (size_t)l * n, (long long)accStride, (long long)n};
        B.cRows = c->ns + 1;
    }
    B.epi = 1;
    B.ein = RowPtr{acc, (long long)accStride, (long long)n};
    B.eout = RowPtr{out0, (long long)(out1 - out0), (long long)n};
    if (T) {
        B.tA0 = T[0];
        B.tA1 = T[1];
        B.tB0 = T[2];
        B.tB1 = T[3];
    } else {
        B.eadd = RowPtr{d0, (long long)(d1 - d0), (long long)n};
    }
    B.k = devConst(d, k1, l);
    B.kS = devConst(d, k1S, l);
    B.k2 = devConst(d, qlinv, l);
    B.k2S = devConst(d, k2S, l);
    epiAddInto(d, B, ea, 2, l);
    nttRows(d, B, 0);
}

void sfp_moddown_rescale(sfp_dev* d, uint64_t* out0, uint64_t* out1, const uint64_t* d0,
                         const uint64_t* d1, uint64_t* acc, size_t accStride, uint32_t ell,
                         uint32_t K, uint32_t Lq, const sfp_conv* c, const uint64_t* pinv,
                         const uint64_t* pmod, const uint64_t* qlinv, uint64_t* scr, int rowDone) {
    moddownRescaleCore(d, out0, out1, d0, d1, nullptr, acc, accStride, ell, K, Lq, c, pinv, pmod, qlinv, scr,
                       rowDone);
}

static int multRelinRescaleCore(sfp_dev* d, uint64_t* out0, uint64_t* out1, const uint64_t* a0, const uint64_t* a1,
                                const uint64_t* b0, const uint64_t* b1, uint32_t ell, uint32_t K, uint32_t Lq,
                                uint32_t alpha, const sfp_conv* const* convs, const uint64_t* key, const sfp_conv* c,
                                const uint64_t* pinv, const uint64_t* pmod, const uint64_t* qlinv, uint64_t* acc,
                                uint64_t* ext, uint64_t* scr, const EpiAdd& ea) {
    const uint32_t beta = (ell + alpha - 1) / alpha;
    if (!ksFuse() || d->n <= (uint32_t)kNttTile) return -1;
    if (ell < 2 || beta > (uint32_t)kMaxConvJobs || ell + K > SFP_MAX_LIMBS) {
        record(d, "mult_relin_rescale (too many digits / limbs)", hipErrorInvalidValue);
        return 0;
    }
    const uint64_t* T[4] = {a0, a1, b0, b1};
    modupInnerCore(d, acc, acc + (size_t)(ell + K) * d->n, a1, b1, ell, K, Lq, alpha, convs, key, nullptr, nullptr,
                   T, pmod[ell - 1], 0, ell - 1, ext, scr);
    moddownRescaleCore(d, out0, out1, nullptr, nullptr, T, acc, (size_t)(ell + K) * d->n, ell, K, Lq, c, pinv, pmod,
                       qlinv, scr, 1, ea);
    return 0;
}

int sfp_mult_relin_rescale(sfp_dev* d, uint64_t* out0, uint64_t* out1, const uint64_t* a0, const uint64_t* a1,
                           const uint64_t* b0, const uint64_t* b1, uint32_t ell, uint32_t K, uint32_t Lq,
                           uint32_t alpha, const sfp_conv* const* convs, const uint64_t* key, const sfp_conv* c,
                           const uint64_t* pinv, const uint64_t* pmod, const uint64_t* qlinv, uint64_t* acc,
                           uint64_t* ext, uint64_t* scr) {
    return multRelinRescaleCore(d, out0, out1, a0, a1, b0, b1, ell, K, Lq, alpha, convs, key, c, pinv, pmod, qlinv,
                                acc, ext, scr, EpiAdd{});
}

static const uint64_t* cstBoth(const uint64_t* cst, uint32_t rows, uint64_t* buf) {
    if (!cst) return nullptr;
    for (uint32_t i = 0; i < rows; ++i) {
        buf[i] = cst[i];
        buf[rows + i] = 0;
    }
    return buf;
}

int sfp_mult_relin_rescale_add(sfp_dev* d, uint64_t* out0, uint64_t* out1, const uint64_t* a0, const uint64_t* a1,
                               const uint64_t* b0, const uint64_t* b1, uint32_t ell, uint32_t K, uint32_t Lq,
                               uint32_t alpha, const sfp_conv* const* convs, const uint64_t* key, const sfp_conv* c,
                               const uint64_t* pinv, const uint64_t* pmod, const uint64_t* qlinv, uint64_t* acc,
                               uint64_t* ext, uint64_t* scr, const uint64_t* r0, const uint64_t* r1, int sign,
                               const uint64_t* cst) {
    uint64_t kb[2 * SFP_MAX_LIMBS];
    if (ell < 2 || ell > SFP_MAX_LIMBS) return -1;
    return multRelinRescaleCore(d, out0, out1, a0, a1, b0, b1, ell, K, Lq, alpha, convs, key, c, pinv, pmod, qlinv,
                                acc, ext, scr, EpiAdd{r0, r1, sign, cstBoth(cst, ell - 1, kb)});
}

int sfp_moddown_rescale_add(sfp_dev* d, uint64_t* out0, uint64_t* out1, const uint64_t* d0, const uint64_t* d1,
                            uint64_t* acc, size_t accStride, uint32_t ell, uint32_t K, uint32_t Lq,
                            const sfp_conv* c, const uint64_t* pinv, const uint64_t* pmod, const uint64_t* qlinv,
                            uint64_t* scr, int rowDone, const uint64_t* r0, const uint64_t* r1, int sign,
                            const uint64_t* cst) {
    uint64_t kb[2 * SFP_MAX_LIMBS];
    if (ell < 2 || ell > SFP_MAX_LIMBS) return -1;
    moddownRescaleCore(d, out0, out1, d0, d1, nullptr, acc, accStride, ell, K, Lq, c, pinv, pmod, qlinv, scr,
                       rowDone, EpiAdd{r0, r1, sign, cstBoth(cst, ell - 1, kb)});
    return 0;
}

void sfp_sample_uniform(sfp_dev* d, uint64_t* p, sfp_limbs m, uint64_t seed) {
    if (!limbsOk(d, m, "uniform")) return;
    const size_t total = (size_t)m.count * d->n;
    SFP_GO(k_uniform, dim3(ewGrid(total)), dim3(kThreads), p, m, seed, d->bar,
                       d->logn);
    checkLaunch(d, "uniform");
}

void sfp_load_i64(sfp_dev* d, uint64_t* p, const int64_t* c, sfp_limbs m) {
    if (!limbsOk(d, m, "load_i64")) return;
    syncAll(d);
    std::memcpy(d->bounce, c, (size_t)d->n * 8);
    SFP_GO(k_load_i64, dim3(ewGrid(d->n)), dim3(kThreads), p,
                       (const int64_t*)d->bounce, m, d->bar, d->logn);
    checkLaunch(d, "load_i64");
}

int sfp_sample_small(sfp_dev* d, uint64_t* p, size_t stride, uint32_t count, const uint64_t* seeds,
                     const uint32_t* kinds, sfp_limbs m) {
// ... 557 lines not shown
```

sorting-fhe_amd/csrc/prims.h:

```cpp
#pragma once
#include <stddef.h>
#include <stdint.h>

#ifdef __cplusplus
extern "C" {
#endif

#define SFP_MAX_LIMBS 96
#define SFP_MAX_WSUM 80

typedef struct sfp_dev sfp_dev;

typedef struct {
    uint32_t count;
    uint32_t split;
    uint32_t pbase;
    uint32_t base;
    uint32_t stride;
} sfp_limbs;

static inline uint32_t sfp_prime_of(sfp_limbs m, uint32_t i) {
    const uint32_t st = m.stride ? m.stride : 1;
    return i < m.split ? m.base + i * st : m.pbase + (i - m.split) * st;
}
// ... 108 lines not shown

void sfp_moddown2(sfp_dev* d, uint64_t* out0, uint64_t* out1, uint64_t* acc, size_t acc_stride,
                  uint32_t ell, uint32_t K, uint32_t Lq, const sfp_conv* c, const uint64_t* pinv,
                  int add0, int add1, uint64_t* scratch, int row_done);

void sfp_ks_inner_fold(sfp_dev* d, uint64_t* acc0, uint64_t* acc1, const uint64_t* ext,
                       size_t ext_stride, const uint64_t* key, uint32_t beta, uint32_t ell,
                       uint32_t K, uint32_t Lq, const uint64_t* fold0, const uint64_t* fold1,
                       uint64_t fold_k);

void sfp_moddown_rescale(sfp_dev* d, uint64_t* out0, uint64_t* out1, const uint64_t* d0,
                         const uint64_t* d1, uint64_t* acc, size_t acc_stride, uint32_t ell,
                         uint32_t K, uint32_t Lq, const sfp_conv* c, const uint64_t* pinv,
                         const uint64_t* pmod, const uint64_t* qlinv, uint64_t* scratch, int row_done);

int sfp_mult_relin_rescale(sfp_dev* d, uint64_t* out0, uint64_t* out1, const uint64_t* a0, const uint64_t* a1,
                           const uint64_t* b0, const uint64_t* b1, uint32_t ell, uint32_t K, uint32_t Lq,
                           uint32_t alpha, const sfp_conv* const* convs, const uint64_t* key, const sfp_conv* c,
                           const uint64_t* pinv, const uint64_t* pmod, const uint64_t* qlinv, uint64_t* acc,
                           uint64_t* ext, uint64_t* scratch);

#if defined(__GNUC__)
#define SFP_OPTIONAL __attribute__((weak))
#else
#define SFP_OPTIONAL
#endif
SFP_OPTIONAL int sfp_mult_relin_rescale_add(sfp_dev* d, uint64_t* out0, uint64_t* out1, const uint64_t* a0,
                                            const uint64_t* a1, const uint64_t* b0, const uint64_t* b1, uint32_t ell,
                                            uint32_t K, uint32_t Lq, uint32_t alpha, const sfp_conv* const* convs,
                                            const uint64_t* key, const sfp_conv* c, const uint64_t* pinv,
                                            const uint64_t* pmod, const uint64_t* qlinv, uint64_t* acc, uint64_t* ext,
                                            uint64_t* scratch, const uint64_t* r0, const uint64_t* r1, int sign,
                                            const uint64_t* cst);
SFP_OPTIONAL int sfp_moddown_rescale_add(sfp_dev* d, uint64_t* out0, uint64_t* out1, const uint64_t* d0,
                                         const uint64_t* d1, uint64_t* acc, size_t acc_stride, uint32_t ell,
                                         uint32_t K, uint32_t Lq, const sfp_conv* c, const uint64_t* pinv,
                                         const uint64_t* pmod, const uint64_t* qlinv, uint64_t* scratch, int row_done,
                                         const uint64_t* r0, const uint64_t* r1, int sign, const uint64_t* cst);
SFP_OPTIONAL int sfp_rescale_add(sfp_dev* d, uint64_t* out, const uint64_t* in, uint32_t ell, const uint64_t* qlinv,
                                 uint32_t npoly, size_t in_stride, size_t out_stride, const uint64_t* cst);
SFP_OPTIONAL int sfp_mul_const_rescale_add(sfp_dev* d, uint64_t* out, const uint64_t* in, const uint64_t* k,
                                           uint32_t ell, const uint64_t* qlinv, uint32_t npoly, size_t in_stride,
                                           size_t out_stride, const uint64_t* cst);

#define SFP_MAX_CONST_TERMS 4
typedef struct {
    uint32_t ell;
    const uint64_t* k;
    const uint64_t* qlinv;
    uint64_t* out;
    size_t out_stride;
    const uint64_t* cst;
} sfp_const_term;
SFP_OPTIONAL int sfp_const_terms_rescale(sfp_dev* d, const uint64_t* in, size_t in_stride, uint32_t npoly,
                                         const sfp_const_term* t, uint32_t m);

SFP_OPTIONAL int sfp_tie_tensor(sfp_dev* d, uint64_t* d0, uint64_t* d1, uint64_t* d2, const uint64_t* s0,
                                const uint64_t* s1, const uint64_t* w, const uint64_t* k, sfp_limbs m);

SFP_OPTIONAL int sfp_decode_batch(sfp_dev* d, const uint64_t* src, size_t srcStride, uint32_t count, uint32_t nl,
                                  uint32_t slots, const double* scales, double* out);

void sfp_sample_uniform(sfp_dev* d, uint64_t* p, sfp_limbs m, uint64_t seed);
void sfp_load_i64(sfp_dev* d, uint64_t* p, const int64_t* coeffs, sfp_limbs m);

#define SFP_SMALL_TERNARY 0u
// ... 93 lines not shown
```

sorting-fhe_amd/python/sfhe.py:

```python
from __future__ import annotations

import ctypes as C
import os
from typing import Sequence

_HERE = os.path.dirname(os.path.abspath(__file__))
PKG_ROOT = os.path.dirname(_HERE)
REPO_ROOT = os.path.dirname(PKG_ROOT)
PRODUCT_LIB = os.path.join(PKG_ROOT, "build", "libsfhe.so")
ORACLE_LIB = os.path.join(REPO_ROOT, "oracle", "_build", "libsfhe_oracle.so")

SFHE_OK = 0
HESTD_128_CLASSIC = 0
HESTD_NOTSET = 3

ABI_SYMBOLS = [
    "sfhe_abi_version", "sfhe_last_error", "sfhe_backend", "sfhe_params_default",
    "sfhe_context_create", "sfhe_context_destroy", "sfhe_keygen", "sfhe_rotate_keygen",
    "sfhe_context_info", "sfhe_context_primes", "sfhe_set_plaintext_cache", "sfhe_set_quiet",
    "sfhe_sync", "sfhe_op_stats", "sfhe_encrypt", "sfhe_decrypt", "sfhe_ct_free",
    "sfhe_ct_clone", "sfhe_ct_info", "sfhe_ct_set_slots", "sfhe_ct_download", "sfhe_eval_add",
    "sfhe_eval_sub", "sfhe_eval_add_const", "sfhe_eval_mult_const", "sfhe_eval_mult_plain",
    "sfhe_eval_mult", "sfhe_eval_rotate", "sfhe_eval_rotate_sum", "sfhe_eval_chebyshev", "sfhe_sign", "sfhe_compare",
    "sfhe_direct_sort_params", "sfhe_doubled_sinc_coeffs", "sfhe_sorter_create",
    "sfhe_sorter_destroy", "sfhe_sorter_sort", "sfhe_sorter_rank", "sfhe_sorter_place",
    "sfhe_decompose", "sfhe_kernel_timing", "sfhe_kernel_timing_read",
    "sfhe_comm_uid", "sfhe_shard_rccl", "sfhe_shard_host", "sfhe_pool_bytes", "sfhe_live_contexts",
    "sfhe_serialize_lanes", "sfhe_stack_stats", "sfhe_comm_stats_reset", "sfhe_comm_stats", "sfhe_sorter_graph_nodes", "sfhe_sorter_create_rot",
    "sfhe_sorter_sort_hybrid1", "sfhe_hybrid1_params", "sfhe_sorter_graph_ntt_time",
    "sfhe_sorter_graph_family_time",
    "sfhe_sorter_sort_hybrid", "sfhe_hybrid_params", "sfhe_sorter_place_2n",
    "sfhe_bootstrap_setup", "sfhe_bootstrap_depth", "sfhe_bootstrap",
    "sfhe_sorter_sort_bitonic", "sfhe_kway_sort", "sfhe_kway_params",
    "sfhe_save", "sfhe_load", "sfhe_ct_save", "sfhe_ct_load",
    "sfhe_kway_create", "sfhe_kway_run", "sfhe_kway_destroy", "sfhe_kway_graph_nodes", "sfhe_kway_graph_family_time", "sfhe_shard_tail",
    "sfhe_key_rows",
    "sfhe_groups_rccl", "sfhe_groups_host", "sfhe_groups",
    "sfhe_encode_counts", "sfhe_bootstrap_graphs",
    "sfhe_decrypt_batch", "sfhe_decode_counts",
    "sfhe_encrypt_batch", "sfhe_sample_counts",
    "sfhe_sorter_sort_stable", "sfhe_sorter_rank_stable", "sfhe_tie_counts",
    "sfhe_const_term_counts",
]


class SfheError(RuntimeError):
    pass


class Params(C.Structure):
    _fields_ = [
        ("mult_depth", C.c_uint32),
        ("scaling_mod_size", C.c_uint32),
        ("first_mod_size", C.c_uint32),
        ("batch_size", C.c_uint32),
        ("ring_dim", C.c_uint32),
        ("security_level", C.c_int32),
        ("num_large_digits", C.c_uint32),
        ("device", C.c_int32),
        ("seed", C.c_uint64),
        ("scaling_technique", C.c_int32),
    ]


_VP = C.c_void_p
_PVP = C.POINTER(C.c_void_p)
_U32 = C.c_uint32
_PU32 = C.POINTER(C.c_uint32)
_SZ = C.c_size_t
_PSZ = C.POINTER(C.c_size_t)
_PD = C.POINTER(C.c_double)
_PI32 = C.POINTER(C.c_int32)
_PU64 = C.POINTER(C.c_uint64)

_AG = C.CFUNCTYPE(None, C.c_void_p, C.c_void_p, C.c_void_p, C.c_size_t)
# ... 60 lines not shown
    "sfhe_ct_save": (C.c_int, [_VP, _VP, C.c_char_p]),
    "sfhe_ct_load": (C.c_int, [_VP, C.c_char_p, _PVP]),
    "sfhe_kway_sort": (C.c_int, [_VP, _VP, C.c_int, C.c_int, C.c_int, C.c_int, C.c_int, _U32, _PVP]),
    "sfhe_kway_params": (C.c_int, [_U32, _PU32, _PU32, _PU32, _PU32, _PI32, _SZ, _PSZ]),
    "sfhe_sorter_graph_ntt_time": (C.c_int, [_VP, C.c_int, _PD, _PU64, _PD]),
    "sfhe_sorter_graph_family_time": (C.c_int, [_VP, C.c_uint32, C.c_int, _PD, _PU64, _PD]),
    "sfhe_kernel_timing": (C.c_int, [_VP, _U32, _U32]),
    "sfhe_serialize_lanes": (C.c_int, [_VP, C.c_int]),
    "sfhe_stack_stats": (C.c_int, [_VP, _PU64, _PU64]),
    "sfhe_comm_stats_reset": (C.c_int, [_VP, C.c_int]),
    "sfhe_comm_stats": (C.c_int, [_VP, _PU64, C.POINTER(C.c_double), C.POINTER(C.c_double)]),
    "sfhe_kernel_timing_read": (C.c_int, [_VP, _U32, _PU64, _PU64, _PD, _PD]),
    "sfhe_decompose": (C.c_int, [_U32, _PI32, _SZ, C.c_int32, C.c_int32, C.c_int, _PI32, _PI32, _SZ, _PSZ]),
    "sfhe_comm_uid": (C.c_int, [_VP]),
    "sfhe_pool_bytes": (C.c_int, [_VP, _PU64]),
    "sfhe_live_contexts": (C.c_int, []),
    "sfhe_shard_rccl": (C.c_int, [_VP, C.c_int, C.c_int, _VP]),
    "sfhe_shard_host": (C.c_int, [_VP, C.c_int, C.c_int, _AG, _BC, _VP]),
    "sfhe_shard_tail": (C.c_int, [_VP, _PU32]),
    "sfhe_key_rows": (C.c_int, [_VP, _PU32]),
    "sfhe_groups_rccl": (C.c_int, [_VP, C.c_int, C.c_int, _VP]),
    "sfhe_groups_host": (C.c_int, [_VP, C.c_int, C.c_int, _AG, _VP]),
    "sfhe_groups": (C.c_int, [_VP, C.POINTER(C.c_int), C.POINTER(C.c_int)]),
    "sfhe_encode_counts": (C.c_int, [_VP, _PU64, _PU64]),
    "sfhe_bootstrap_graphs": (C.c_int, [_VP, _PU64]),
    "sfhe_decrypt_batch": (C.c_int, [_VP, C.POINTER(_VP), _SZ, _PD, _SZ, _PSZ]),
    "sfhe_decode_counts": (C.c_int, [_VP, _PU64, _PU64]),
    "sfhe_encrypt_batch": (C.c_int, [_VP, _PD, _SZ, _PSZ, _SZ, _U32, _PU32, C.POINTER(_VP)]),
    "sfhe_sample_counts": (C.c_int, [_VP, _PU64, _PU64]),
    "sfhe_sorter_sort_stable": (C.c_int, [_VP, _VP, C.c_int, C.c_int, C.c_int, _PVP]),
    "sfhe_sorter_rank_stable": (C.c_int, [_VP, _VP, C.c_int, C.c_int, C.c_int, _PVP]),
    "sfhe_tie_counts": (C.c_int, [_VP, _PU64, _PU64]),
    "sfhe_const_term_counts": (C.c_int, [_VP, _PU64, _PU64, _PU64]),
}

_libs: dict = {}


def lib_path(backend: str = "hip") -> str:
    return os.environ.get("SFHE_PRODUCT_LIB", PRODUCT_LIB) if backend == "hip" else ORACLE_LIB


ABI_VERSION = 3


def load(backend: str = "hip"):
    if backend in _libs:
        return _libs[backend]
    path = lib_path(backend)
    if not os.path.exists(path):
        raise SfheError(
            f"{backend} library not built: {path} is missing "
            f"(run `make -C sorting-fhe_amd` for the HIP product, `make -C oracle` for the oracle)")
    lib = C.CDLL(path)
    for name, (res, args) in _SIGS.items():
        f = getattr(lib, name)
        f.restype = res
        f.argtypes = args
    if lib.sfhe_abi_version() != ABI_VERSION:
        raise SfheError(f"{path}: C ABI version {lib.sfhe_abi_version()}, this binding speaks {ABI_VERSION} "
                        "(rebuild the library or use the matching sfhe.py)")
    _libs[backend] = lib
    return lib


def _darr(v: Sequence[float]):
    a = (C.c_double * len(v))(*[float(x) for x in v])
    return a


class Engine:

    def __init__(self, backend: str = "hip", *, mult_depth: int, ring_dim: int = 0,
                 batch_size: int = 0, scaling_mod_size: int = 40, first_mod_size: int = 60,
                 secure: bool = False, num_large_digits: int = 0, seed: int = 0x5EED5EED2025,
                 device: int = 0, rotations: Sequence[int] = (), keygen: bool = True,
                 scaling: str = "FLEXIBLEAUTOEXT", shard=None, groups=None):
        self.lib = load(backend)
        self.backend = backend
        p = Params()
        self.lib.sfhe_params_default(C.byref(p))
        p.mult_depth = mult_depth
        p.ring_dim = ring_dim
        p.batch_size = batch_size
        p.scaling_mod_size = scaling_mod_size
        p.first_mod_size = first_mod_size
        p.security_level = HESTD_128_CLASSIC if secure else HESTD_NOTSET
        p.num_large_digits = num_large_digits
# ... 198 lines not shown

    def decrypt(self, ct: "Ct") -> list:
        n = ct.slots
        buf = (C.c_double * n)()
        self._chk(self.lib.sfhe_decrypt(self.ctx, ct.h, buf, n, None))
        return list(buf)

    def decrypt_batch(self, cts: Sequence["Ct"]) -> list:
        cts = list(cts)
        if not cts:
            return []
        stride = max(c.slots for c in cts)
        hs = (_VP * len(cts))(*[c.h for c in cts])
        buf = (C.c_double * (stride * len(cts)))()
        lens = (C.c_size_t * len(cts))()
        self._chk(self.lib.sfhe_decrypt_batch(self.ctx, hs, len(cts), buf, stride, lens))
        return [list(buf[k * stride:k * stride + lens[k]]) for k in range(len(cts))]

    def decode_counts(self):
        d, h = C.c_uint64(), C.c_uint64()
        self._chk(self.lib.sfhe_decode_counts(self.ctx, C.byref(d), C.byref(h)))
        return d.value, h.value

    def tie_counts(self):
        f, c = C.c_uint64(), C.c_uint64()
        self._chk(self.lib.sfhe_tie_counts(self.ctx, C.byref(f), C.byref(c)))
        return f.value, c.value

    def const_term_counts(self):
        m, s1, c = C.c_uint64(), C.c_uint64(), C.c_uint64()
        self._chk(self.lib.sfhe_const_term_counts(self.ctx, C.byref(m), C.byref(s1), C.byref(c)))
        return m.value, s1.value, c.value

    def add(self, a, b):
        return self._new(self.lib.sfhe_eval_add, self.ctx, a.h, b.h)

    def sub(self, a, b):
        return self._new(self.lib.sfhe_eval_sub, self.ctx, a.h, b.h)

    def add_const(self, a, k: float):
        return self._new(self.lib.sfhe_eval_add_const, self.ctx, a.h, float(k))

    def mult_const(self, a, k: float):
        return self._new(self.lib.sfhe_eval_mult_const, self.ctx, a.h, float(k))

    def mult_plain(self, a, values: Sequence[float], slots: int = 0):
        return self._new(self.lib.sfhe_eval_mult_plain, self.ctx, a.h, _darr(values), len(values), slots)

    def mult(self, a, b):
        return self._new(self.lib.sfhe_eval_mult, self.ctx, a.h, b.h)

    def rotate(self, a, r: int):
        return self._new(self.lib.sfhe_eval_rotate, self.ctx, a.h, int(r))

    def rotate_sum(self, cts, rots):
        hs = (_VP * len(cts))(*[c.h for c in cts])
        rs = (C.c_int32 * len(rots))(*[int(r) for r in rots])
        return self._new(self.lib.sfhe_eval_rotate_sum, self.ctx, hs, rs, len(cts))

    def bootstrap_setup(self, level_budget=(5, 5), slots: int = 0):
        self._chk(self.lib.sfhe_bootstrap_setup(self.ctx, level_budget[0], level_budget[1], slots))

    def bootstrap_depth(self, level_budget=(5, 5), slots: int = 0) -> int:
        v = C.c_uint32()
        self._chk(self.lib.sfhe_bootstrap_depth(self.ctx, level_budget[0], level_budget[1], slots, C.byref(v)))
        return v.value
# ... 353 lines not shown
```

Baseline: 2.040 million cmp/s.

## Fuse operand doubling into mult-relin-rescale kernels and defer sign-poly adds

Adds `twice` variants of the fused multiply-relinearize-rescale primitives that double operand A inside the kernel. Chebyshev power generation (2*T_a*T_b - T_c) and the giant-step powers no longer need a separate doubled ciphertext. The odd-polynomial evaluator in sign also attaches the lower-half sum to the product as a deferred epilogue add. Together these are meant to remove standalone add kernels and extra ciphertext buffers on the comparison path, at the cost of more kernel variants and a fallback path that materialises the doubling.

Result: no change. 2.053 million cmp/s (median of 6 runs) (+0.6%).

```diff
diff --git a/include/sfhe.h b/include/sfhe.h
--- a/include/sfhe.h
+++ b/include/sfhe.h
@@ -60,6 +60,7 @@
 int sfhe_decode_counts(sfhe_ctx* c, uint64_t* device, uint64_t* host);
 int sfhe_tie_counts(sfhe_ctx* c, uint64_t* fused, uint64_t* composed);
 int sfhe_const_term_counts(sfhe_ctx* c, uint64_t* merged, uint64_t* single, uint64_t* composed);
+int sfhe_mul_twice_counts(sfhe_ctx* c, uint64_t* fused, uint64_t* materialised);
 int sfhe_sample_counts(sfhe_ctx* c, uint64_t* device, uint64_t* host);
 int sfhe_pool_bytes(sfhe_ctx* c, uint64_t* bytes);
 int sfhe_live_contexts(void);
@@ -99,6 +100,8 @@
 int sfhe_eval_mult(sfhe_ctx* c, const sfhe_ct* a, const sfhe_ct* b, sfhe_ct** out);
 int sfhe_eval_rotate(sfhe_ctx* c, const sfhe_ct* a, int32_t r, sfhe_ct** out);
 int sfhe_eval_rotate_sum(sfhe_ctx* c, const sfhe_ct* const* a, const int32_t* r, size_t count, sfhe_ct** out);
+int sfhe_eval_mult_many_add(sfhe_ctx* c, const sfhe_ct* const* a, const sfhe_ct* const* b, const sfhe_ct* const* r,
+                            const int* sign, const double* k, const uint8_t* twice, size_t count, sfhe_ct** out);
 int sfhe_bootstrap_setup(sfhe_ctx* c, uint32_t budget_c2s, uint32_t budget_s2c, uint32_t slots);
 int sfhe_bootstrap_depth(sfhe_ctx* c, uint32_t budget_c2s, uint32_t budget_s2c, uint32_t slots, uint32_t* depth);
 int sfhe_bootstrap(sfhe_ctx* c, const sfhe_ct* a, uint32_t iterations, uint32_t precision, sfhe_ct** out);
diff --git a/sorting-fhe_amd/csrc/algo/sign.cpp b/sorting-fhe_amd/csrc/algo/sign.cpp
--- a/sorting-fhe_amd/csrc/algo/sign.cpp
+++ b/sorting-fhe_amd/csrc/algo/sign.cpp
@@ -74,6 +74,7 @@
         uint32_t Lp;
         int hi, lo;
         Ct prod, out;
+        bool summed = false;
     };
     std::vector<Node> nodes;
     std::vector<Ct> pw;
@@ -86,7 +87,7 @@
         return std::max(natural(half), pwLevel(OddPoly::powIndex(half))) + 1;
     }
     int build(const double* c, size_t cnt, uint32_t want) {
-        Node nd{c, cnt, 0, 0, -1, -1, nullptr, nullptr};
+        Node nd{c, cnt, 0, 0, -1, -1, nullptr, nullptr, false};
         if (cnt == 1) {
             nd.Lp = std::max(L + 1, want);
         } else {
@@ -125,7 +126,12 @@
                     power = &it->second;
                 }
                 if (!nodes[nd.hi].out) continue;
-                nd.prod = cc->EvalMult(nodes[nd.hi].out, *power);
+                if (nodes[nd.lo].out)
+                    nd.prod = cc->EvalMultDeferredAdd(nodes[nd.hi].out, *power,
+                                                      CryptoContextImpl<DCRTPoly>::MultAddend{nodes[nd.lo].out, 1, 0.0},
+                                                      &nd.summed);
+                else
+                    nd.prod = cc->EvalMult(nodes[nd.hi].out, *power);
                 prods.push_back(nd.prod);
             }
             const bool first = ready == 0;
@@ -143,7 +149,8 @@
             }
             for (const auto& key : align) aligned[key] = cc->AdjustLevel(pw[key.first], key.second);
             for (Node& nd : nodes)
-                if (nd.cnt > 1 && !nd.out && nd.prod && nodes[nd.lo].out) nd.out = cc->EvalAdd(nodes[nd.lo].out, nd.prod);
+                if (nd.cnt > 1 && !nd.out && nd.prod && nodes[nd.lo].out)
+                    nd.out = nd.summed ? nd.prod : cc->EvalAdd(nodes[nd.lo].out, nd.prod);
         }
         return nodes[root].out;
     }
diff --git a/sorting-fhe_amd/csrc/capi.cpp b/sorting-fhe_amd/csrc/capi.cpp
--- a/sorting-fhe_amd/csrc/capi.cpp
+++ b/sorting-fhe_amd/csrc/capi.cpp
@@ -378,6 +378,12 @@
     return SFHE_OK;
 }
 
+int sfhe_mul_twice_counts(sfhe_ctx* c, uint64_t* fused, uint64_t* materialised) {
+    REQUIRE(c && fused && materialised, "null argument");
+    c->cc->MulTwiceCounts(fused, materialised);
+    return SFHE_OK;
+}
+
 void sfhe_ct_free(sfhe_ct* ct) { delete ct; }
 
 int sfhe_ct_clone(const sfhe_ct* ct, sfhe_ct** out) {
@@ -444,6 +450,37 @@
         std::vector<Ciphertext<DCRTPoly>> v;
         for (size_t k = 0; k < count; ++k) v.push_back(a[k]->ct);
         *out = wrap(c->cc->EvalRotateSum(v, std::vector<int32_t>(r, r + count)));
+    });
+}
+int sfhe_eval_mult_many_add(sfhe_ctx* c, const sfhe_ct* const* a, const sfhe_ct* const* b, const sfhe_ct* const* r,
+                            const int* sign, const double* k, const uint8_t* twice, size_t count, sfhe_ct** out) {
+    REQUIRE(c && a && b && out && count, "null argument");
+    for (size_t i = 0; i < count; ++i) REQUIRE(a[i] && b[i], "null argument");
+    return guard([&] {
+        using CC = CryptoContextImpl<DCRTPoly>;
+        std::vector<Ciphertext<DCRTPoly>> as, bs;
+        std::vector<CC::MultAddend> adds(count);
+        for (size_t i = 0; i < count; ++i) {
+            as.push_back(a[i]->ct);
+            bs.push_back(b[i]->ct);
+            c->cc->Settle(as.back());
+            c->cc->Settle(bs.back());
+            if (r && r[i]) {
+                adds[i].r = r[i]->ct;
+                c->cc->Settle(adds[i].r);
+                adds[i].sign = sign ? sign[i] : 1;
+            }
+            adds[i].c = k ? k[i] : 0.0;
+            adds[i].twiceA = twice && twice[i];
+        }
+        struct Hold {
+            SfheContextState* s;
+            explicit Hold(SfheContextState* s_) : s(s_) { ++s->lazyHold; }
+            ~Hold() { --s->lazyHold; }
+        } hold(c->cc->state());
+        auto res = count == 1 ? std::vector<Ciphertext<DCRTPoly>>{c->cc->EvalMultAdd(as[0], bs[0], adds[0])}
+                              : c->cc->EvalMultManyAdd(as, bs, adds);
+        for (size_t i = 0; i < count; ++i) out[i] = wrap(res[i]);
     });
 }
 int sfhe_bootstrap_setup(sfhe_ctx* c, uint32_t budget_c2s, uint32_t budget_s2c, uint32_t slots) {
diff --git a/sorting-fhe_amd/csrc/core/chebyshev.cpp b/sorting-fhe_amd/csrc/core/chebyshev.cpp
--- a/sorting-fhe_amd/csrc/core/chebyshev.cpp
+++ b/sorting-fhe_amd/csrc/core/chebyshev.cpp
@@ -71,9 +71,12 @@
         for (uint32_t half = 1; half < k; half *= 2) {
             const uint32_t lo = half + 1, hi = std::min(k, 2 * half);
             std::vector<Ct> as, bs;
+            std::vector<char> tw;
             for (uint32_t j = lo; j <= hi; ++j) {
-                as.push_back(doubled(j / 2));
-                bs.push_back(j % 2 == 0 ? T[j / 2] : T[j / 2 + 1]);
+                const Ct& b = j % 2 == 0 ? T[j / 2] : T[j / 2 + 1];
+                tw.push_back(cc->MulTwiceFusable(T[j / 2], b));
+                as.push_back(tw.back() ? T[j / 2] : doubled(j / 2));
+                bs.push_back(b);
             }
             uint32_t top = 0;
             for (size_t i = 0; i < as.size(); ++i) top = std::max(top, std::max(as[i]->GetLevel(), bs[i]->GetLevel()) + 1);
@@ -82,6 +85,7 @@
                 for (uint32_t j = lo; j <= hi; ++j) {
                     const uint32_t lv = std::max(as[j - lo]->GetLevel(), bs[j - lo]->GetLevel()) + 1;
                     adds.push_back(j % 2 == 0 ? Addend{nullptr, 1, -1.0} : Addend{atLevel(1, lv), -1, 0.0});
+                    adds.back().twiceA = tw[j - lo];
                 }
                 if (psWaves()) {
                     auto ts = cc->EvalMultManyAdd(as, bs, adds);
@@ -93,9 +97,13 @@
             }
             std::vector<Ct> prods;
             if (psWaves()) {
-                prods = cc->EvalMultMany(as, bs);
+                prods = cc->EvalMultMany(as, bs, &tw);
             } else {
-                for (size_t i = 0; i < as.size(); ++i) prods.push_back(cc->EvalMult(as[i], bs[i]));
+                for (size_t i = 0; i < as.size(); ++i) {
+                    Addend none;
+                    none.twiceA = tw[i];
+                    prods.push_back(tw[i] ? cc->EvalMultAdd(as[i], bs[i], none) : cc->EvalMult(as[i], bs[i]));
+                }
             }
             for (uint32_t j = lo; j <= hi; ++j) {
                 const Ct& prod = prods[j - lo];
@@ -386,14 +394,15 @@
         auto it = giant.find(i);
         if (it != giant.end()) return it->second;
         const Ct& half = power(M / 2);
-        const Ct twice = cc->EvalAdd(half, half);
-        return giant[i] = cc->EvalMultAdd(twice, half, Addend{nullptr, 1, -1.0});
+        Addend minusOne{nullptr, 1, -1.0};
+        minusOne.twiceA = cc->MulTwiceFusable(half, half);
+        return giant[i] = cc->EvalMultAdd(minusOne.twiceA ? half : cc->DoubledOperand(half), half, minusOne);
     }
 
     const Ct& doubled(uint32_t j) {
         auto it = twice.find(j);
         if (it != twice.end()) return it->second;
-        return twice[j] = cc->EvalAdd(T[j], T[j]);
+        return twice[j] = cc->DoubledOperand(T[j]);
     }
 
     const Ct& alignedPower(uint32_t M, uint32_t level) {
@@ -462,8 +471,13 @@
     if (!std::getenv("SFHE_PS_DEBUG")) return;
     uint64_t sums = 0, consts = 0, pairs = 0;
     cc->FusedSumCounts(&sums, &consts, &pairs);
-    std::fprintf(stderr, "PSFMA %s | fused sums %llu | fused constants %llu | paired weighted sums %llu\n", where,
-                 (unsigned long long)sums, (unsigned long long)consts, (unsigned long long)pairs);
+    uint64_t twF = 0, twM = 0;
+    cc->MulTwiceCounts(&twF, &twM);
+    std::fprintf(stderr,
+                 "PSFMA %s | fused sums %llu | fused constants %llu | paired weighted sums %llu | doublings fused %llu "
+                 "stored %llu\n",
+                 where, (unsigned long long)sums, (unsigned long long)consts, (unsigned long long)pairs,
+                 (unsigned long long)twF, (unsigned long long)twM);
 }
 
 }
diff --git a/sorting-fhe_amd/csrc/core/context.cpp b/sorting-fhe_amd/csrc/core/context.cpp
--- a/sorting-fhe_amd/csrc/core/context.cpp
+++ b/sorting-fhe_amd/csrc/core/context.cpp
@@ -907,11 +907,56 @@
     }
 
     static Ct multRelinRescale(CC* cc, const uint64_t* a0, const uint64_t* a1, const uint64_t* b0,
-                               const uint64_t* b1, uint32_t level, uint32_t slots, Fma* f = nullptr) {
+                               const uint64_t* b1, uint32_t level, uint32_t slots, Fma* f = nullptr,
+                               bool twice = false) {
         SfheContextState* s = cc->st.get();
         const uint32_t ell = s->ellOf(level);
         if (ell < 2) SFHE_THROW("no levels left to rescale (multiplicative depth exhausted)");
         const size_t pw = s->polyWords(level);
+        DeviceBufferPtr dbl;
+        if (twice) {
+            if (!s->shardAt(ell) && sfp_mult_relin_rescale_twice && sfp_mult_relin_rescale_add_twice) {
+                const DeviceBufferPtr& key = s->relinFor(ell);
+                const int tier = key->ksTier;
+                const uint32_t n = s->n, K = s->Kof(tier), beta = (ell + s->alpha - 1) / s->alpha;
+                const size_t stride = (size_t)(ell + K) * n;
+                Ct out = newCt(cc, level + 1, slots);
+                auto acc = s->alloc(2 * stride);
+                auto ext = s->alloc(stride * beta);
+                auto scratch = s->alloc((size_t)2 * ell * n);
+                auto& convs = modupConv(cc, ell, tier);
+                int rc = -1;
+                if (f && *f) {
+                    rc = sfp_mult_relin_rescale_add_twice(s->dev, out->c0, out->c1, a0, a1, b0, b1, ell, K, s->Lq,
+                                                          s->alpha, convs.data(), key->ptr, s->moddownConvOf(tier),
+                                                          s->pInvModQof(tier), s->pModQof(tier),
+                                                          s->qInvTable[ell].data(), acc->ptr, ext->ptr, scratch->ptr,
+                                                          f->r0, f->r1, f->sign, f->cst);
+                    if (rc == 0) f->done = true;
+                } else {
+                    rc = sfp_mult_relin_rescale_twice(s->dev, out->c0, out->c1, a0, a1, b0, b1, ell, K, s->Lq, s->alpha,
+                                                      convs.data(), key->ptr, s->moddownConvOf(tier),
+                                                      s->pInvModQof(tier), s->pModQof(tier), s->qInvTable[ell].data(),
+                                                      acc->ptr, ext->ptr, scratch->ptr);
+                }
+                if (rc == 0) {
+                    s->twiceFused++;
+                    s->stats.keyswitch++;
+                    s->stats.rescale++;
+                    s->countBytes((3.0 * ell + 2.0 * beta * (ell + K)) * n * 8);
+                    s->countBytes(4.0 * ell * n * 8);
+                    return out;
+                }
+            }
+            dbl = s->alloc(2 * pw);
+            sfp_add(s->dev, dbl->ptr, a0, a0, s->qmap(ell));
+            sfp_add(s->dev, dbl->ptr + pw, a1, a1, s->qmap(ell));
+            s->twiceMaterialised++;
+            s->stats.add++;
+            s->countBytes(6.0 * ell * s->n * 8);
+            a0 = dbl->ptr;
+            a1 = dbl->ptr + pw;
+        }
         if (!s->shardAt(ell)) {
             const DeviceBufferPtr& key = s->relinFor(ell);
             const int tier = key->ksTier;
@@ -953,9 +998,11 @@
 
     static std::vector<Ct> multRelinRescaleMany(CC* cc, const std::vector<const CiphertextImpl<DCRTPoly>*>& a,
                                                 const std::vector<const CiphertextImpl<DCRTPoly>*>& b, uint32_t level,
-                                                const std::vector<uint32_t>& slots, std::vector<Fma>* fs = nullptr) {
+                                                const std::vector<uint32_t>& slots, std::vector<Fma>* fs = nullptr,
+                                                const std::vector<char>* tw = nullptr) {
         SfheContextState* s = cc->st.get();
         const size_t cnt = a.size();
+        const bool twPrims = sfp_mult_relin_rescale_twice && sfp_mult_relin_rescale_add_twice;
         const uint32_t ell = s->ellOf(level);
         std::vector<Ct> out(cnt);
         if (ell < 2) SFHE_THROW("no levels left to rescale (multiplicative depth exhausted)");
@@ -976,7 +1023,25 @@
                 bs.lane((uint32_t)done);
                 Fma* f = fs && (*fs)[done] ? &(*fs)[done] : nullptr;
                 int rc = -1;
-                if (f && sfp_mult_relin_rescale_add) {
+                if (tw && (*tw)[done]) {
+                    if (!twPrims) break;
+                    if (f) {
+                        rc = sfp_mult_relin_rescale_add_twice(
+                            s->dev, out[done]->c0, out[done]->c1, a[done]->c0, a[done]->c1, b[done]->c0, b[done]->c1,
+                            ell, K, s->Lq, s->alpha, convs.data(), key->ptr, s->moddownConvOf(tier),
+                            s->pInvModQof(tier), s->pModQof(tier), s->qInvTable[ell].data(), acc->ptr, ext->ptr,
+                            scratch->ptr, f->r0, f->r1, f->sign, f->cst);
+                        if (rc == 0) f->done = true;
+                    } else {
+                        rc = sfp_mult_relin_rescale_twice(
+                            s->dev, out[done]->c0, out[done]->c1, a[done]->c0, a[done]->c1, b[done]->c0, b[done]->c1,
+                            ell, K, s->Lq, s->alpha, convs.data(), key->ptr, s->moddownConvOf(tier),
+                            s->pInvModQof(tier), s->pModQof(tier), s->qInvTable[ell].data(), acc->ptr, ext->ptr,
+                            scratch->ptr);
+                    }
+                    if (rc != 0) break;
+                    s->twiceFused++;
+                } else if (f && sfp_mult_relin_rescale_add) {
                     rc = sfp_mult_relin_rescale_add(s->dev, out[done]->c0, out[done]->c1, a[done]->c0, a[done]->c1,
                                                     b[done]->c0, b[done]->c1, ell, K, s->Lq, s->alpha, convs.data(),
                                                     key->ptr, s->moddownConvOf(tier), s->pInvModQof(tier),
@@ -984,7 +1049,7 @@
                                                     scratch->ptr, f->r0, f->r1, f->sign, f->cst);
                     if (rc == 0) f->done = true;
                 }
-                if (rc != 0)
+                if (rc != 0 && !(tw && (*tw)[done]))
                     rc = sfp_mult_relin_rescale(s->dev, out[done]->c0, out[done]->c1, a[done]->c0, a[done]->c1,
                                                 b[done]->c0, b[done]->c1, ell, K, s->Lq, s->alpha, convs.data(),
                                                 key->ptr, s->moddownConvOf(tier), s->pInvModQof(tier),
@@ -1000,7 +1065,7 @@
         }
         for (size_t i = done; i < cnt; ++i)
             out[i] = multRelinRescale(cc, a[i]->c0, a[i]->c1, b[i]->c0, b[i]->c1, level, slots[i],
-                                      fs ? &(*fs)[i] : nullptr);
+                                      fs ? &(*fs)[i] : nullptr, tw && (*tw)[i]);
         return out;
     }
 
@@ -1710,14 +1775,36 @@
     DeviceBufferPtr pa, pb;
     const uint64_t *a0, *a1, *b0, *b1;
     uint32_t level, slots;
+    DeviceBufferPtr pr;
+    const uint64_t *r0 = nullptr, *r1 = nullptr;
     void sync(SfheContextState* s) override {
         s->dep(pa.get());
         s->dep(pb.get());
+        if (pr) s->dep(pr.get());
     }
     void run(CCI* cc, CtI& ct, bool pending) override {
         SfheContextState* s = cc->state();
         s->dep(pa.get());
         s->dep(pb.get());
+        if (pr) {
+            if (pending) SFHE_THROW("internal: a product with an attached sum was asked for its pending rows");
+            s->dep(pr.get());
+            SfheInternal::Fma f;
+            f.r0 = r0;
+            f.r1 = r1;
+            auto out = SfheInternal::multRelinRescale(cc, a0, a1, b0, b1, level, slots, &f);
+            const uint32_t l = s->ellOf(level) - 1;
+            if (f.done) {
+                s->fusedSums++;
+            } else {
+                sfp_add(s->dev, out->c0, out->c0, r0, s->qmap(l));
+                sfp_add(s->dev, out->c1, out->c1, r1, s->qmap(l));
+            }
+            s->stats.add++;
+            s->countBytes(6.0 * l * s->n * 8);
+            SfheInternal::adopt(ct, out);
+            return;
+        }
         if (!pending) {
             SfheInternal::adopt(ct, SfheInternal::multRelinRescale(cc, a0, a1, b0, b1, level, slots));
             return;
@@ -2082,18 +2169,22 @@
         std::type_index kind;
         bool pending;
         size_t ct;
-        bool like(const Item& o) const { return level == o.level && kind == o.kind && pending == o.pending; }
+        bool sum;
+        bool like(const Item& o) const {
+            return level == o.level && kind == o.kind && pending == o.pending && sum == o.sum;
+        }
     };
     std::vector<Item> items;
     for (size_t i = 0; i < cts.size(); ++i) {
         const auto& c = cts[i];
         if (!c || (!c->def && !(c->pend && !pendingOk[i]))) continue;
         const DeferredOp* d = c->def.get();
+        const auto* dr = dynamic_cast<const DeferredRelin*>(d);
         items.push_back({c->level ? c->level - 1 : 0, d ? std::type_index(typeid(*d)) : std::type_index(typeid(void)),
-                         pendingOk[i] != 0, i});
+                         pendingOk[i] != 0, i, dr && dr->pr});
     }
     std::stable_sort(items.begin(), items.end(), [](const Item& a, const Item& b) {
-        return std::tie(a.level, a.kind, a.pending) < std::tie(b.level, b.kind, b.pending);
+        return std::tie(a.level, a.kind, a.pending, a.sum) < std::tie(b.level, b.kind, b.pending, b.sum);
     });
     const size_t w = batchWidth();
     for (size_t b0 = 0, b1; b0 < items.size(); b0 = b1) {
@@ -2919,12 +3010,26 @@
 }
 
 std::vector<Ciphertext<DCRTPoly>> CryptoContextImpl<DCRTPoly>::EvalMultMany(
-    const std::vector<Ciphertext<DCRTPoly>>& a0, const std::vector<Ciphertext<DCRTPoly>>& b0) {
+    const std::vector<Ciphertext<DCRTPoly>>& a00, const std::vector<Ciphertext<DCRTPoly>>& b0,
+    const std::vector<char>* twiceA) {
     OpLock g(st.get());
     SfheContextState* s = st.get();
-    if (a0.size() != b0.size()) SFHE_THROW("operand count mismatch");
-    const size_t cnt = a0.size();
+    if (a00.size() != b0.size() || (twiceA && twiceA->size() != a00.size())) SFHE_THROW("operand count mismatch");
+    const size_t cnt = a00.size();
     std::vector<Ciphertext<DCRTPoly>> out(cnt);
+    std::vector<Ciphertext<DCRTPoly>> a0(a00);
+    std::vector<char> tw(cnt, 0);
+    for (size_t i = 0; twiceA && i < cnt; ++i)
+        if ((*twiceA)[i]) {
+            tw[i] = cnt >= 2 && MulTwiceFusable(a0[i], b0[i]);
+            if (!tw[i]) a0[i] = cnt >= 2 ? DoubledOperand(a0[i]) : a0[i];
+        }
+    if (cnt == 1 && twiceA && (*twiceA)[0]) {
+        MultAddend none;
+        none.twiceA = true;
+        out[0] = EvalMultAdd(a0[0], b0[0], none);
+        return out;
+    }
     if (cnt < 2 || !SfheInternal::fusedRescale()) {
         for (size_t i = 0; i < cnt; ++i) out[i] = EvalMult(a0[i], b0[i]);
         return out;
@@ -2948,7 +3053,8 @@
             pb.push_back(B[k].get());
             slots.push_back(std::max(A[k]->slots, B[k]->slots));
         }
-        auto r = SfheInternal::multRelinRescaleMany(this, pa, pb, A[i]->level, slots);
+        const std::vector<char> tws(tw.begin() + i, tw.begin() + j);
+        auto r = SfheInternal::multRelinRescaleMany(this, pa, pb, A[i]->level, slots, nullptr, &tws);
         for (size_t k = i; k < j; ++k) out[k] = SfheInternal::traced(this, r[k - i], "EvalMult");
         i = j;
     }
@@ -2986,7 +3092,27 @@
                                                              const Ciphertext<DCRTPoly>& b0,
                                                              const MultAddend& add) {
     OpLock g(st.get());
-    if (!multAddFusable(a0, b0, add)) return addAfter(this, EvalMult(a0, b0), add);
+    if (add.twiceA) {
+        MultAddend rest = add;
+        rest.twiceA = false;
+        if (!MulTwiceFusable(a0, b0)) return EvalMultAdd(DoubledOperand(a0), b0, rest);
+        if (!multAddFusable(a0, b0, add)) {
+            SfheContextState* s = st.get();
+            SfheInternal::deps(s, {&a0, &b0});
+            auto a = a0, b = b0;
+            SfheInternal::align(this, a, b);
+            s->stats.tensor++;
+            s->countBytes(7.0 * s->ellOf(a->level) * s->n * 8);
+            auto prod = SfheInternal::traced(
+                this,
+                SfheInternal::multRelinRescale(this, a->c0, a->c1, b->c0, b->c1, a->level,
+                                               std::max(a->slots, b->slots), nullptr, true),
+                "EvalMult");
+            return addAfter(this, prod, rest);
+        }
+    } else if (!multAddFusable(a0, b0, add)) {
+        return addAfter(this, EvalMult(a0, b0), add);
+    }
     SfheContextState* s = st.get();
     SfheInternal::deps(s, {&a0, &b0, &add.r});
     auto a = a0, b = b0;
@@ -3006,24 +3132,32 @@
         f.cst = k.data();
     }
     auto out = SfheInternal::traced(
-        this, SfheInternal::multRelinRescale(this, a->c0, a->c1, b->c0, b->c1, a->level, slots, &f), "EvalMult");
+        this, SfheInternal::multRelinRescale(this, a->c0, a->c1, b->c0, b->c1, a->level, slots, &f, add.twiceA),
+        "EvalMult");
     if (!f.done) return addAfter(this, out, add);
     SfheInternal::countFused(s, add, ell - 1);
     return out;
 }
 
 std::vector<Ciphertext<DCRTPoly>> CryptoContextImpl<DCRTPoly>::EvalMultManyAdd(
-    const std::vector<Ciphertext<DCRTPoly>>& a0, const std::vector<Ciphertext<DCRTPoly>>& b0,
+    const std::vector<Ciphertext<DCRTPoly>>& a00, const std::vector<Ciphertext<DCRTPoly>>& b0,
     const std::vector<MultAddend>& adds) {
     OpLock g(st.get());
     SfheContextState* s = st.get();
-    if (a0.size() != b0.size() || a0.size() != adds.size()) SFHE_THROW("operand count mismatch");
-    const size_t cnt = a0.size();
+    if (a00.size() != b0.size() || a00.size() != adds.size()) SFHE_THROW("operand count mismatch");
+    const size_t cnt = a00.size();
     std::vector<Ciphertext<DCRTPoly>> out(cnt);
     if (cnt < 2) {
-        for (size_t i = 0; i < cnt; ++i) out[i] = EvalMultAdd(a0[i], b0[i], adds[i]);
+        for (size_t i = 0; i < cnt; ++i) out[i] = EvalMultAdd(a00[i], b0[i], adds[i]);
         return out;
     }
+    std::vector<Ciphertext<DCRTPoly>> a0(a00);
+    std::vector<char> tw(cnt, 0);
+    for (size_t i = 0; i < cnt; ++i)
+        if (adds[i].twiceA) {
+            tw[i] = MulTwiceFusable(a0[i], b0[i]);
+            if (!tw[i]) a0[i] = DoubledOperand(a0[i]);
+        }
     if (!psFma() || !SfheInternal::fusedRescale() || SfheInternal::lazy(s)) {
         out = EvalMultMany(a0, b0);
         for (size_t i = 0; i < cnt; ++i) out[i] = addAfter(this, out[i], adds[i]);
@@ -3065,7 +3199,8 @@
                 f.cst = ks[k - i].data();
             }
         }
-        auto r = SfheInternal::multRelinRescaleMany(this, pa, pb, level, slots, &fs);
+        const std::vector<char> tws(tw.begin() + i, tw.begin() + j);
+        auto r = SfheInternal::multRelinRescaleMany(this, pa, pb, level, slots, &fs, &tws);
         for (size_t k = i; k < j; ++k) {
             out[k] = SfheInternal::traced(this, r[k - i], "EvalMult");
             if (fs[k - i].done)
@@ -3076,6 +3211,63 @@
         i = j;
     }
     return out;
+}
+
+Ciphertext<DCRTPoly> CryptoContextImpl<DCRTPoly>::EvalMultDeferredAdd(const Ciphertext<DCRTPoly>& a0,
+                                                                     const Ciphertext<DCRTPoly>& b0,
+                                                                     const MultAddend& add, bool* attached) {
+    OpLock g(st.get());
+    SfheContextState* s = st.get();
+    *attached = false;
+    const bool can = signFma() && psFma() && SfheInternal::fusedRescale() && SfheInternal::lazy(s) && s->relinKey &&
+                     sfp_mult_relin_rescale_add && add.r && add.sign >= 0 && add.c == 0.0 && !add.twiceA &&
+                     !SfheInternal::isLazy(add.r);
+    if (!can) return EvalMult(a0, b0);
+    SfheInternal::deps(s, {&a0, &b0});
+    auto a = a0, b = b0;
+    SfheInternal::align(this, a, b);
+    const uint32_t level = a->level, ell = s->ellOf(level);
+    const auto& r = add.r;
+    if (ell < 2 || s->shardAt(ell) || level + 1 > s->L || r->level != level + 1 || r->scale != s->scale[level + 1] ||
+        r->c1 - r->c0 != (ptrdiff_t)s->polyWords(level + 1))
+        return EvalMult(a, b);
+    s->stats.tensor++;
+    s->countBytes(7.0 * ell * s->n * 8);
+    auto op = std::make_shared<DeferredRelin>();
+    op->pa = a->buf;
+    op->pb = b->buf;
+    op->a0 = a->c0;
+    op->a1 = a->c1;
+    op->b0 = b->c0;
+    op->b1 = b->c1;
+    op->level = level;
+    op->slots = std::max(std::max(a->slots, b->slots), r->slots);
+    op->pr = r->buf;
+    op->r0 = r->c0;
+    op->r1 = r->c1;
+    *attached = true;
+    return SfheInternal::deferredCt(this, level + 1, op->slots, op);
+}
+
+bool CryptoContextImpl<DCRTPoly>::MulTwiceFusable(const Ciphertext<DCRTPoly>& a, const Ciphertext<DCRTPoly>& b) const {
+    SfheContextState* s = st.get();
+    if (!mulTwice() || !psFma() || !SfheInternal::fusedRescale() || SfheInternal::lazy(s) || !s->relinKey) return false;
+    if (!sfp_mult_relin_rescale_twice || !sfp_mult_relin_rescale_add_twice) return false;
+    if (!a || !b || SfheInternal::isLazy(a) || SfheInternal::isLazy(b)) return false;
+    if (a->level < b->level) return false;
+    const uint32_t ell = s->ellOf(a->level);
+    return ell >= 2 && !s->shardAt(ell) && a->level + 1 <= s->L;
+}
+
+Ciphertext<DCRTPoly> CryptoContextImpl<DCRTPoly>::DoubledOperand(const Ciphertext<DCRTPoly>& a) {
+    OpLock g(st.get());
+    st->twiceMaterialised++;
+    return EvalAdd(a, a);
+}
+
+void CryptoContextImpl<DCRTPoly>::MulTwiceCounts(uint64_t* fused, uint64_t* materialised) const {
+    *fused = st->twiceFused;
+    *materialised = st->twiceMaterialised;
 }
 
 Ciphertext<DCRTPoly> CryptoContextImpl<DCRTPoly>::EvalMultAddPlain(
diff --git a/sorting-fhe_amd/csrc/core/openfhe.h b/sorting-fhe_amd/csrc/core/openfhe.h
--- a/sorting-fhe_amd/csrc/core/openfhe.h
+++ b/sorting-fhe_amd/csrc/core/openfhe.h
@@ -312,12 +312,19 @@
     Ciphertext<DCRTPoly> EvalSquare(const Ciphertext<DCRTPoly>& a);
     Ciphertext<DCRTPoly> EvalTieTerm(const Ciphertext<DCRTPoly>& s, const Plaintext& W, double k);
     std::vector<Ciphertext<DCRTPoly>> EvalMultMany(const std::vector<Ciphertext<DCRTPoly>>& a,
-                                                   const std::vector<Ciphertext<DCRTPoly>>& b);
+                                                   const std::vector<Ciphertext<DCRTPoly>>& b,
+                                                   const std::vector<char>* twiceA = nullptr);
     struct MultAddend {
         Ciphertext<DCRTPoly> r;
         int sign = 1;
         double c = 0.0;
+        bool twiceA = false;
     };
+    bool MulTwiceFusable(const Ciphertext<DCRTPoly>& a, const Ciphertext<DCRTPoly>& b) const;
+    Ciphertext<DCRTPoly> DoubledOperand(const Ciphertext<DCRTPoly>& a);
+    void MulTwiceCounts(uint64_t* fused, uint64_t* materialised) const;
+    Ciphertext<DCRTPoly> EvalMultDeferredAdd(const Ciphertext<DCRTPoly>& a, const Ciphertext<DCRTPoly>& b,
+                                             const MultAddend& add, bool* attached);
     Ciphertext<DCRTPoly> EvalMultAdd(const Ciphertext<DCRTPoly>& a, const Ciphertext<DCRTPoly>& b,
                                      const MultAddend& add);
     std::vector<Ciphertext<DCRTPoly>> EvalMultManyAdd(const std::vector<Ciphertext<DCRTPoly>>& a,
diff --git a/sorting-fhe_amd/csrc/core/state.h b/sorting-fhe_amd/csrc/core/state.h
--- a/sorting-fhe_amd/csrc/core/state.h
+++ b/sorting-fhe_amd/csrc/core/state.h
@@ -151,6 +151,7 @@
     uint64_t captureEpoch = 0, epochCount = 0;
     uint32_t lazyHold = 0;
     uint64_t fusedSums = 0, fusedConsts = 0, pairedWsums = 0;
+    uint64_t twiceFused = 0, twiceMaterialised = 0;
     std::set<uint64_t> abandonedEpochs;
     std::vector<std::pair<uint64_t*, size_t>> capAllocs;
     std::unordered_map<uint64_t*, bool> graphOwned;
@@ -243,6 +244,16 @@
     return !v || *v != '0';
 }
 
+inline bool mulTwice() {
+    const char* v = std::getenv("SFHE_MUL_TWICE");
+    return !v || *v != '0';
+}
+
+inline bool signFma() {
+    const char* v = std::getenv("SFHE_SIGN_FMA");
+    return v && *v == '1';
+}
+
 class OpLock {
   public:
     explicit OpLock(SfheContextState* s) : s_(s), g_(s->opMu) {
diff --git a/sorting-fhe_amd/csrc/hip/prims_hip.hip b/sorting-fhe_amd/csrc/hip/prims_hip.hip
--- a/sorting-fhe_amd/csrc/hip/prims_hip.hip
+++ b/sorting-fhe_amd/csrc/hip/prims_hip.hip
@@ -662,6 +662,7 @@
     };
     const struct MdColArgs* md;
     uint32_t esumNeg;
+    uint32_t aTwice;
 };
 
 template <class T, int NG>
@@ -709,6 +710,14 @@
 #else
 #define NTT_MARK(i)
 #endif
+
+__device__ __forceinline__ ulonglong2 twiceMod(ulonglong2 x, u64 q) {
+    x.x += x.x;
+    x.y += x.y;
+    x.x = x.x >= q ? x.x - q : x.x;
+    x.y = x.y >= q ? x.y - q : x.y;
+    return x;
+}
 
 template <bool INV, bool COL, int LE, int TILE, int NG = 1, bool CONV = false>
 __global__ __launch_bounds__(TILE >> LE) void k_ntt(const RowGroupSet<NG> GS, const sf_barrett* __restrict__ bar,
@@ -893,6 +902,7 @@
             if (cp) *reinterpret_cast<ulonglong2*>(cp + g) = x;
             if (pre) {
                 const ulonglong2 m = mr[k];
+                if (G.aTwice) x = twiceMod(x, q);
                 x.x = bmul(x.x, m.x, LB);
                 x.y = bmul(x.y, m.y, LB);
             }
@@ -1026,14 +1036,16 @@
             if (ead || tens) {
                 ulonglong2 o;
                 if (tens) {
-                    const ulonglong2 a0 = *reinterpret_cast<const ulonglong2*>(G.tA0 + trow + g);
+                    ulonglong2 a0 = *reinterpret_cast<const ulonglong2*>(G.tA0 + trow + g);
                     const ulonglong2 b0 = *reinterpret_cast<const ulonglong2*>(G.tB0 + trow + g);
+                    if (G.aTwice) a0 = twiceMod(a0, q);
                     if (pp == 0) {
                         o.x = bmul(a0.x, b0.x, EB);
                         o.y = bmul(a0.y, b0.y, EB);
                     } else {
-                        const ulonglong2 a1 = *reinterpret_cast<const ulonglong2*>(G.tA1 + trow + g);
+                        ulonglong2 a1 = *reinterpret_cast<const ulonglong2*>(G.tA1 + trow + g);
                         const ulonglong2 b1 = *reinterpret_cast<const ulonglong2*>(G.tB1 + trow + g);
+                        if (G.aTwice) a1 = twiceMod(a1, q);
                         Acc t{0, 0}, u{0, 0};
                         macc(t, a0.x, b1.x);
                         macc(t, a1.x, b0.x);
@@ -1370,6 +1382,7 @@
     uint32_t invFrom;
     const u64 *itw, *itwS;
     const double* itwD;
+    uint32_t aTwice;
 };
 
 template <int LE, int TILE, int NG = 1>
@@ -1470,6 +1483,7 @@
                     ulonglong2 x = *reinterpret_cast<const ulonglong2*>(src + e);
                     if (mul) {
                         const ulonglong2 m = *reinterpret_cast<const ulonglong2*>(mul + e);
+                        if (A.aTwice) x = twiceMod(x, q);
                         x.x = bmul(x.x, m.x, B);
                         x.y = bmul(x.y, m.y, B);
                     }
@@ -1581,8 +1595,12 @@
             if (fold) {
                 if (A.fa0) {
                     const size_t ro = (size_t)t * n + rowOff + e;
-                    const ulonglong2 x0 = *reinterpret_cast<const ulonglong2*>(A.fa0 + ro);
-                    const ulonglong2 x1 = *reinterpret_cast<const ulonglong2*>(A.fa1 + ro);
+                    ulonglong2 x0 = *reinterpret_cast<const ulonglong2*>(A.fa0 + ro);
+                    ulonglong2 x1 = *reinterpret_cast<const ulonglong2*>(A.fa1 + ro);
+                    if (A.aTwice) {
+                        x0 = twiceMod(x0, q);
+                        x1 = twiceMod(x1, q);
+                    }
                     const ulonglong2 y0 = *reinterpret_cast<const ulonglong2*>(A.fb0 + ro);
                     const ulonglong2 y1 = *reinterpret_cast<const ulonglong2*>(A.fb1 + ro);
                     if constexpr (FP) {
@@ -5549,7 +5567,7 @@
                            uint32_t ell, uint32_t K, uint32_t Lq, uint32_t alpha, const sfp_conv* const* convs,
                            const uint64_t* key, const uint64_t* fold0, const uint64_t* fold1,
                            const uint64_t* const* T, uint64_t foldK, int accum, uint32_t invFrom, uint64_t* ext,
-                           uint64_t* scr, int phases = 3) {
+                           uint64_t* scr, int phases = 3, bool aTwice = false) {
     const uint32_t n = d->n;
     const uint32_t beta = (ell + alpha - 1) / alpha;
     const long long stride = (long long)(ell + K) * n;
@@ -5558,6 +5576,7 @@
     A.src = RowPtr{in, 0, (long long)n};
     A.dst = RowPtr{scr, 0, (long long)n};
     if (inMul) A.pre = RowPtr{inMul, 0, (long long)n};
+    A.aTwice = inMul && aTwice ? 1u : 0u;
     RowGroup B = rowsOf(beta, ell + K, sfp_limbs{ell + K, ell, Lq, 0});
     B.src = B.dst = RowPtr{ext, stride, (long long)n};
     B.skipEll = ell;
@@ -5597,6 +5616,7 @@
         a.fb1 = T[3];
     }
     a.foldK = foldK;
+    a.aTwice = aTwice ? 1u : 0u;
     a.ell = ell;
     a.Lq = Lq;
     a.alpha = alpha;
@@ -5857,7 +5877,8 @@
 static void moddownRescaleCore(sfp_dev* d, uint64_t* out0, uint64_t* out1, const uint64_t* d0, const uint64_t* d1,
                                const uint64_t* const* T, uint64_t* acc, size_t accStride, uint32_t ell, uint32_t K,
                                uint32_t Lq, const sfp_conv* c, const uint64_t* pinv, const uint64_t* pmod,
-                               const uint64_t* qlinv, uint64_t* scr, int rowDone, const EpiAdd& ea = EpiAdd{}) {
+                               const uint64_t* qlinv, uint64_t* scr, int rowDone, const EpiAdd& ea = EpiAdd{},
+                               bool aTwice = false) {
     const uint32_t n = d->n, l = ell - 1;
     if (ell < 2 || ell > SFP_MAX_LIMBS || !c || c->ns > (uint32_t)kMaxConvSrc || c->nt < ell ||
         !limbsOk(d, sfp_limbs{K + 1, 1, Lq, l}, "moddown_rescale")) {
@@ -5972,6 +5993,7 @@
         B.tA1 = T[1];
         B.tB0 = T[2];
         B.tB1 = T[3];
+        B.aTwice = aTwice ? 1u : 0u;
     } else {
         B.eadd = RowPtr{d0, (long long)(d1 - d0), (long long)n};
     }
@@ -5995,7 +6017,7 @@
                                 const uint64_t* b0, const uint64_t* b1, uint32_t ell, uint32_t K, uint32_t Lq,
                                 uint32_t alpha, const sfp_conv* const* convs, const uint64_t* key, const sfp_conv* c,
                                 const uint64_t* pinv, const uint64_t* pmod, const uint64_t* qlinv, uint64_t* acc,
-                                uint64_t* ext, uint64_t* scr, const EpiAdd& ea) {
+                                uint64_t* ext, uint64_t* scr, const EpiAdd& ea, bool aTwice = false) {
     const uint32_t beta = (ell + alpha - 1) / alpha;
     if (!ksFuse() || d->n <= (uint32_t)kNttTile) return -1;
     if (ell < 2 || beta > (uint32_t)kMaxConvJobs || ell + K > SFP_MAX_LIMBS) {
@@ -6004,9 +6026,9 @@
     }
     const uint64_t* T[4] = {a0, a1, b0, b1};
     modupInnerCore(d, acc, acc + (size_t)(ell + K) * d->n, a1, b1, ell, K, Lq, alpha, convs, key, nullptr, nullptr,
-                   T, pmod[ell - 1], 0, ell - 1, ext, scr);
+                   T, pmod[ell - 1], 0, ell - 1, ext, scr, 3, aTwice);
     moddownRescaleCore(d, out0, out1, nullptr, nullptr, T, acc, (size_t)(ell + K) * d->n, ell, K, Lq, c, pinv, pmod,
-                       qlinv, scr, 1, ea);
+                       qlinv, scr, 1, ea, aTwice);
     return 0;
 }
 
@@ -6038,6 +6060,28 @@
     if (ell < 2 || ell > SFP_MAX_LIMBS) return -1;
     return multRelinRescaleCore(d, out0, out1, a0, a1, b0, b1, ell, K, Lq, alpha, convs, key, c, pinv, pmod, qlinv,
                                 acc, ext, scr, EpiAdd{r0, r1, sign, cstBoth(cst, ell - 1, kb)});
+}
+
+int sfp_mult_relin_rescale_twice(sfp_dev* d, uint64_t* out0, uint64_t* out1, const uint64_t* a0, const uint64_t* a1,
+                                 const uint64_t* b0, const uint64_t* b1, uint32_t ell, uint32_t K, uint32_t Lq,
+                                 uint32_t alpha, const sfp_conv* const* convs, const uint64_t* key, const sfp_conv* c,
+                                 const uint64_t* pinv, const uint64_t* pmod, const uint64_t* qlinv, uint64_t* acc,
+                                 uint64_t* ext, uint64_t* scr) {
+    return multRelinRescaleCore(d, out0, out1, a0, a1, b0, b1, ell, K, Lq, alpha, convs, key, c, pinv, pmod, qlinv,
+                                acc, ext, scr, EpiAdd{}, true);
+}
+
+int sfp_mult_relin_rescale_add_twice(sfp_dev* d, uint64_t* out0, uint64_t* out1, const uint64_t* a0,
+                                     const uint64_t* a1, const uint64_t* b0, const uint64_t* b1, uint32_t ell,
+                                     uint32_t K, uint32_t Lq, uint32_t alpha, const sfp_conv* const* convs,
+                                     const uint64_t* key, const sfp_conv* c, const uint64_t* pinv,
+                                     const uint64_t* pmod, const uint64_t* qlinv, uint64_t* acc, uint64_t* ext,
+                                     uint64_t* scr, const uint64_t* r0, const uint64_t* r1, int sign,
+                                     const uint64_t* cst) {
+    uint64_t kb[2 * SFP_MAX_LIMBS];
+    if (ell < 2 || ell > SFP_MAX_LIMBS) return -1;
+    return multRelinRescaleCore(d, out0, out1, a0, a1, b0, b1, ell, K, Lq, alpha, convs, key, c, pinv, pmod, qlinv,
+                                acc, ext, scr, EpiAdd{r0, r1, sign, cstBoth(cst, ell - 1, kb)}, true);
 }
 
 int sfp_moddown_rescale_add(sfp_dev* d, uint64_t* out0, uint64_t* out1, const uint64_t* d0, const uint64_t* d1,
diff --git a/sorting-fhe_amd/csrc/prims.h b/sorting-fhe_amd/csrc/prims.h
--- a/sorting-fhe_amd/csrc/prims.h
+++ b/sorting-fhe_amd/csrc/prims.h
@@ -164,6 +164,19 @@
                                             const uint64_t* pmod, const uint64_t* qlinv, uint64_t* acc, uint64_t* ext,
                                             uint64_t* scratch, const uint64_t* r0, const uint64_t* r1, int sign,
                                             const uint64_t* cst);
+SFP_OPTIONAL int sfp_mult_relin_rescale_twice(sfp_dev* d, uint64_t* out0, uint64_t* out1, const uint64_t* a0,
+                                              const uint64_t* a1, const uint64_t* b0, const uint64_t* b1, uint32_t ell,
+                                              uint32_t K, uint32_t Lq, uint32_t alpha, const sfp_conv* const* convs,
+                                              const uint64_t* key, const sfp_conv* c, const uint64_t* pinv,
+                                              const uint64_t* pmod, const uint64_t* qlinv, uint64_t* acc,
+                                              uint64_t* ext, uint64_t* scratch);
+SFP_OPTIONAL int sfp_mult_relin_rescale_add_twice(sfp_dev* d, uint64_t* out0, uint64_t* out1, const uint64_t* a0,
+                                                  const uint64_t* a1, const uint64_t* b0, const uint64_t* b1,
+                                                  uint32_t ell, uint32_t K, uint32_t Lq, uint32_t alpha,
+                                                  const sfp_conv* const* convs, const uint64_t* key, const sfp_conv* c,
+                                                  const uint64_t* pinv, const uint64_t* pmod, const uint64_t* qlinv,
+                                                  uint64_t* acc, uint64_t* ext, uint64_t* scratch, const uint64_t* r0,
+                                                  const uint64_t* r1, int sign, const uint64_t* cst);
 SFP_OPTIONAL int sfp_moddown_rescale_add(sfp_dev* d, uint64_t* out0, uint64_t* out1, const uint64_t* d0,
                                          const uint64_t* d1, uint64_t* acc, size_t acc_stride, uint32_t ell,
                                          uint32_t K, uint32_t Lq, const sfp_conv* c, const uint64_t* pinv,
diff --git a/sorting-fhe_amd/python/sfhe.py b/sorting-fhe_amd/python/sfhe.py
--- a/sorting-fhe_amd/python/sfhe.py
+++ b/sorting-fhe_amd/python/sfhe.py
@@ -40,7 +40,7 @@
     "sfhe_decrypt_batch", "sfhe_decode_counts",
     "sfhe_encrypt_batch", "sfhe_sample_counts",
     "sfhe_sorter_sort_stable", "sfhe_sorter_rank_stable", "sfhe_tie_counts",
-    "sfhe_const_term_counts",
+    "sfhe_const_term_counts", "sfhe_mul_twice_counts", "sfhe_eval_mult_many_add",
 ]
 
 
@@ -167,6 +167,9 @@
     "sfhe_sorter_rank_stable": (C.c_int, [_VP, _VP, C.c_int, C.c_int, C.c_int, _PVP]),
     "sfhe_tie_counts": (C.c_int, [_VP, _PU64, _PU64]),
     "sfhe_const_term_counts": (C.c_int, [_VP, _PU64, _PU64, _PU64]),
+    "sfhe_mul_twice_counts": (C.c_int, [_VP, _PU64, _PU64]),
+    "sfhe_eval_mult_many_add": (C.c_int, [_VP, C.POINTER(_VP), C.POINTER(_VP), C.POINTER(_VP), C.POINTER(C.c_int),
+                                          _PD, C.POINTER(C.c_uint8), C.c_size_t, C.POINTER(_VP)]),
 }
 
 _libs: dict = {}
@@ -189,6 +192,8 @@
             f"(run `make -C sorting-fhe_amd` for the HIP product, `make -C oracle` for the oracle)")
     lib = C.CDLL(path)
     for name, (res, args) in _SIGS.items():
+        if name in ("sfhe_mul_twice_counts", "sfhe_eval_mult_many_add") and not hasattr(lib, name):
+            continue
         f = getattr(lib, name)
         f.restype = res
         f.argtypes = args
@@ -453,6 +458,23 @@
         self._chk(self.lib.sfhe_const_term_counts(self.ctx, C.byref(m), C.byref(s1), C.byref(c)))
         return m.value, s1.value, c.value
 
+    def mul_twice_counts(self):
+        f, m = C.c_uint64(), C.c_uint64()
+        self._chk(self.lib.sfhe_mul_twice_counts(self.ctx, C.byref(f), C.byref(m)))
+        return f.value, m.value
+
+    def mult_many_add(self, a, b, r=None, sign=None, k=None, twice=None):
+        n = len(a)
+        ha = (_VP * n)(*[x.h for x in a])
+        hb = (_VP * n)(*[x.h for x in b])
+        hr = (_VP * n)(*[(x.h if x is not None else None) for x in (r or [None] * n)])
+        sg = (C.c_int * n)(*[int(x) for x in (sign or [1] * n)])
+        kk = (C.c_double * n)(*[float(x) for x in (k or [0.0] * n)])
+        tw = (C.c_uint8 * n)(*[1 if x else 0 for x in (twice or [0] * n)])
+        outs = (_VP * n)()
+        self._chk(self.lib.sfhe_eval_mult_many_add(self.ctx, ha, hb, hr, sg, kk, tw, n, outs))
+        return [Ct(self, _VP(h)) for h in outs]
+
     def add(self, a, b):
         return self._new(self.lib.sfhe_eval_add, self.ctx, a.h, b.h)
 
```
